# cosmodesi/desilike

Measured on AMD Instinct MI355X. Metric: log-likelihood evals/sec (full-shape P_ell, 3x40 bins), higher is better.
Workload: dtype f64; 1 GPU; BASELINE configs[1]: ShapeFit+Kaiser P_ell ell=(0,2,4) x 40 k-bins, dense window 120x1200 (n_kin=400/ell), 120x120 precision, 1024 batched param points per GPU per step; batch_per_gpu=1024, n_params=6, parallelism=walkers x1, collective=none, ranks=1

## Files before the change

### desilike_amd/csrc/dl_api.hip

```cpp
#include <hip/hip_runtime.h>
#include <chrono>
#include <thread>

#include <algorithm>
#include <cstdio>
#include <cstdlib>
#include <string>
#include <vector>

#include "../../include/desilike_amd.h"
#include "dl_host.hpp"
#include "dl_kernels.h"
#include "dl_ens_fold.h"
#include "dl_prior.h"

static thread_local std::string g_last_error;
void dl_set_last_error(const char* msg) { g_last_error = msg ? msg : ""; }

struct dl_ctx {
    int device = 0;
    int n_params = 0, n_obs = 0, n_data = 0;
    int n_white = 0;
    int N_pad = 0, K_pad = 0, K_live = 0, max_n_t = 0;
    bool any_transform = false;
// ... 389 lines not shown
        if (dl_upload(ctx, &dev, gf)) { dl_destroy(ctx); return 1; }
        ctx->gfrag_dev.push_back(dev);
    }
    ctx->obs_kernarg.resize(ctx->n_obs);
    for (int i = 0; i < ctx->n_obs; ++i) { ctx->obs[i].rebase(ctx->arena_dev); ctx->obs_kernarg[i] = ctx->obs[i].dev; }
    if (dl_upload(ctx, &ctx->obs_array_dev, ctx->obs_kernarg)) { dl_destroy(ctx); return 1; }
    {
        size_t nbytes = (16384 / 32 + 8 + 64) * sizeof(int32_t);
        if (hipMalloc((void**)&ctx->gemm_counters, nbytes) != hipSuccess || hipMemset(ctx->gemm_counters, 0, nbytes) != hipSuccess) { dl_fail(ctx, "dl_create: counter allocation failed"); dl_destroy(ctx); return 1; }
        ctx->step_ready = ctx->gemm_counters + (16384 / 32 + 8);
    }
    {
        std::vector<double> frag((size_t)ctx->N_pad * ctx->K_pad);
        const int nks = ctx->K_pad / 4;
        for (int nt = 0; nt < ctx->N_pad / 16; ++nt)
            for (int ks = 0; ks < nks; ++ks)
                for (int lane = 0; lane < 64; ++lane)
                    frag[((size_t)nt * nks + ks) * 64 + lane] = wt_white[(size_t)(16 * nt + (lane & 15)) * ctx->K_pad + 4 * ks + (lane >> 4)];
        if (dl_upload(ctx, &ctx->wt_frag_dev, frag)) { dl_destroy(ctx); return 1; }
    }
    if (dl_upload(ctx, &ctx->priors_dev, priors) || dl_upload(ctx, &ctx->wt_white_dev, wt_white) ||
        dl_upload(ctx, &ctx->bias_white_dev, bias_white) || dl_upload(ctx, &ctx->wt_full_dev, wt_full) || dl_upload(ctx, &ctx->bias_full_dev, bias_full) ||
        dl_upload(ctx, &ctx->wh_dev, wh) || dl_upload(ctx, &ctx->bias_wh_dev, bias_wh) || dl_upload(ctx, &ctx->flatdata_dev, flatdata) ||
        dl_upload(ctx, &ctx->transform_dev, transform)) {
        dl_destroy(ctx);
        return 1;
    }
    if (hipDeviceSynchronize() != hipSuccess) { dl_fail(ctx, "dl_create: hipDeviceSynchronize failed"); dl_destroy(ctx); return 1; }
    *out = ctx;
    return 0;
}

static double* dl_stk_basis_ws(dl_ctx* ctx, int i) {
    const DlObsDev& d = ctx->obs_kernarg[i];
    if (d.eng[0].type != 2 || ctx->power_ws == nullptr) return nullptr;
    const int64_t ldk = (int64_t)d.stk.n_trunks * d.eng[0].widths[d.eng[0].n_layers];
    return ldk <= (int64_t)(1 + ctx->n_var) * ctx->K_pad ? ctx->power_ws : nullptr;
}

void dl_destroy(dl_ctx* ctx) {
    if (!ctx) return;
    (void)hipSetDevice(ctx->device);
    for (double* p : {ctx->grad_wtT, ctx->grad_zero, ctx->grad_delta, ctx->grad_y, ctx->grad_phys}) if (p) (void)hipFree(p);
    for (double* p : {ctx->fa_resid, ctx->fa_jac, ctx->fa_rows}) if (p) (void)hipFree(p);
    for (double* p : {ctx->ej_basis, ctx->ej_u, ctx->ej_c, ctx->ej_dc, ctx->ej_resid, ctx->ej_rows}) if (p) (void)hipFree(p);
    for (double* p : {ctx->eg_gt, ctx->eg_u, ctx->eg_v, ctx->eg_q, ctx->eg_gb, ctx->eg_wt[0], ctx->eg_wt[1], ctx->eg_wt[2]}) if (p) (void)hipFree(p);
    if (ctx->grad_status) (void)hipFree(ctx->grad_status);
    void* ptrs[] = {ctx->arena_dev, ctx->priors_dev, ctx->wt_white_dev, ctx->wt_frag_dev, ctx->bias_white_dev, ctx->wt_full_dev, ctx->bias_full_dev, ctx->wh_dev,
                    ctx->bias_wh_dev, ctx->flatdata_dev, ctx->transform_dev, ctx->tconst_dev, ctx->power_ws, ctx->delta_ws, ctx->flat_ws, ctx->stencil_ws, ctx->theta_stage, ctx->out_stage,
                    ctx->status_stage, ctx->gemm_counters, ctx->obs_array_dev};
    for (void* p : ptrs) if (p) (void)hipFree(p);
    for (double* p : ctx->gfrag_dev) if (p) (void)hipFree(p);
    for (auto& ob : ctx->obs) if (ob.tns) { dl_tns_destroy(ob.tns); ob.tns = nullptr; }
    if (ctx->feat_ws) (void)hipFree(ctx->feat_ws);
    for (hipEvent_t e : ctx->ev) if (e) (void)hipEventDestroy(e);
    if (ctx->order_event) (void)hipEventDestroy(ctx->order_event);
    if (ctx->host_stage) (void)hipHostFree(ctx->host_stage);
    if (ctx->host_flag) (void)hipHostFree(ctx->host_flag);
    if (ctx->host_event) (void)hipEventDestroy(ctx->host_event);
    if (ctx->host_stream) (void)hipStreamDestroy(ctx->host_stream);
    delete ctx;
}

static bool dl_fisher_emu_in_scope(const dl_ctx* ctx);
static int64_t dl_fisher_emu_per_pass(const dl_ctx* ctx);

int64_t dl_info(const dl_ctx* ctx, const char* key) {
    if (!ctx || !key) return -1;
    std::string k(key);
    if (k == "fisher_analytic_pass") return dl_fisher_emu_in_scope(ctx) ? dl_fisher_emu_per_pass(ctx) : -1;
    if (k == "n_params") return ctx->n_params;
    if (k == "n_data") return ctx->n_data;
    if (k == "n_obs") return ctx->n_obs;
    if (k == "n_in_total") { int64_t t = 0; for (auto& o : ctx->obs) t += o.n_cols(); return t; }
    if (k == "K_pad") return ctx->K_pad;
    if (k == "N_pad") return ctx->N_pad;
    if (k == "n_solved") return ctx->n_solved;
    if (k == "device") return ctx->device;
    for (int i = 0; i < ctx->n_obs; ++i) {
        if (k == "n_in_obs" + std::to_string(i)) return ctx->obs[i].dev.n_in;
        if (k == "n_out_obs" + std::to_string(i)) return ctx->obs[i].n_out;
        if (k == "n_ell_obs" + std::to_string(i)) return ctx->obs[i].dev.n_ell;
        if (k == "n_kin_obs" + std::to_string(i)) return ctx->obs[i].dev.n_kin;
    }
    return -1;
}

static const int64_t DL_CHUNK = 32768;

static int dl_reserve(dl_ctx* ctx, int64_t B) {
    int64_t need = std::min<int64_t>(B, DL_CHUNK);
    if (need <= ctx->cap) return 0;
    need = std::min<int64_t>(std::max<int64_t>(need, 1024), DL_CHUNK);
    if (ctx->cap > 0) DL_HIP_CHECK(ctx, hipDeviceSynchronize());
    for (double** p : {&ctx->power_ws, &ctx->delta_ws, &ctx->flat_ws, &ctx->feat_ws, &ctx->stencil_ws}) if (*p) { (void)hipFree(*p); *p = nullptr; }
    ctx->cap = 0;
    const size_t R = 1 + ctx->n_var;
    DL_HIP_CHECK(ctx, hipMalloc((void**)&ctx->power_ws, (size_t)need * R * ctx->K_pad * sizeof(double)));
    DL_HIP_CHECK(ctx, hipMalloc((void**)&ctx->delta_ws, std::max<size_t>(2 * (size_t)need * R, (size_t)need * R + 16384 + 2048) * ctx->N_pad * sizeof(double)));
    DL_HIP_CHECK(ctx, hipMalloc((void**)&ctx->flat_ws, (size_t)need * ctx->N_pad * sizeof(double)));
    if (ctx->feat_ok) DL_HIP_CHECK(ctx, hipMalloc((void**)&ctx->feat_ws, (size_t)need * ctx->feat_ld * sizeof(double)));
    DL_HIP_CHECK(ctx, hipMalloc((void**)&ctx->stencil_ws, (size_t)need * ctx->n_params * sizeof(double)));
    DL_HIP_CHECK(ctx, hipMemset(ctx->power_ws, 0, (size_t)need * R * ctx->K_pad * sizeof(double)));
    DL_HIP_CHECK(ctx, hipMemset(ctx->delta_ws, 0, std::max<size_t>(2 * (size_t)need * R, (size_t)need * R + 16384 + 2048) * ctx->N_pad * sizeof(double)));
    DL_HIP_CHECK(ctx, hipMemset(ctx->flat_ws, 0, (size_t)need * ctx->N_pad * sizeof(double)));
    if (ctx->feat_ok) DL_HIP_CHECK(ctx, hipMemset(ctx->feat_ws, 0, (size_t)need * ctx->feat_ld * sizeof(double)));
    DL_HIP_CHECK(ctx, hipMemset(ctx->stencil_ws, 0, (size_t)need * ctx->n_params * sizeof(double)));
    DL_HIP_CHECK(ctx, hipDeviceSynchronize());
    ctx->cap = need;
    return 0;
}

static int dl_eval_impl(dl_ctx* ctx, const double* theta_dev, int64_t B, double* loglike_dev, double* logprior_dev, double* flattheory_dev, int32_t* status_dev,
                        double* solved_dev, void* hip_stream, int post_mode, double* hessian_dev = nullptr) {
    if (!ctx) { g_last_error = "dl_eval_batch: null context"; return 1; }
    if (B < 0 || (B > 0 && !theta_dev)) return dl_fail(ctx, "dl_eval_batch: invalid batch");
    if (B == 0) return 0;
    hipStream_t stream = (hipStream_t)hip_stream;
    dl_prof_events.start = dl_prof_events.stop = nullptr;
    DL_HIP_CHECK(ctx, hipSetDevice(ctx->device));
    if (dl_order_streams(ctx, stream)) return 1;
    if (dl_reserve(ctx, B)) return 1;
    const int n = ctx->n_data, P = ctx->n_params, R = 1 + ctx->n_var;
    for (int64_t b0 = 0; b0 < B; b0 += DL_CHUNK) {
        int64_t nb = std::min<int64_t>(DL_CHUNK, B - b0);
        const double* th = theta_dev + (size_t)b0 * P;
        bool prof = ctx->profile && b0 == 0 && (ctx->eval_calls % ctx->prof_every == ctx->prof_every / 2);
        hipEvent_t* ev = prof ? &ctx->ev[(size_t)(ctx->prof_calls % dl_ctx::NPOOL) * 6] : nullptr;
        const int64_t pc = ctx->prof_calls;
        const int only = !ctx->prof_rotate ? -1 : ctx->prof_only;
        if (prof) ctx->prof_phase_of[(size_t)(pc % dl_ctx::NPOOL)] = (int8_t)only;
        auto prof_phase = [&](int k) {
            const bool on = ev && k >= 0 && (only < 0 || only == k);
            dl_prof_events.start = on ? ev[2 * k] : nullptr;
            dl_prof_events.stop = on ? ev[2 * k + 1] : nullptr;
        };
        bool need_flat = ctx->any_transform || flattheory_dev != nullptr;
        const bool feat_path = ctx->feat_ok && !need_flat;
        const bool emu_fused_env = !dl_options().no_emu_fused;
        const bool emu_fused = emu_fused_env || ctx->any_stacked;
        const int64_t chi2_max_rows = dl_options().chi2_max_rows;
        const bool chi2_path = !feat_path && !ctx->any_transform && ctx->n_solved == 0 && nb <= chi2_max_rows;
        const int xcd_local = dl_options().xcd_local;
        const bool chi2_fused_env_early = dl_options().chi2_fused;
        const bool chi2_fused_early = chi2_fused_env_early && !ctx->priors_general;
        const int xcd_block = !xcd_local ? 0 : chi2_path ? (chi2_fused_early ? 32 : dl_chi2_gemm_row_tile(nb, ctx->N_pad)) : (xcd_local > 1 && !feat_path && !ctx->any_transform && ctx->n_solved == 0 && ctx->N_pad == 128) ? 64 : 0;
        const bool step_kernel_allowed = dl_options().step_kernel;
        if (step_kernel_allowed && chi2_path && !need_flat && ctx->n_obs == 1 && !ctx->priors_general && ctx->K_pad % 128 == 0 &&
            dl_step_lds_bytes(ctx->obs_kernarg[0], nb, ctx->N_pad) != 0) {
            prof_phase(0);
            dl_launch_step(ctx->obs_kernarg[0], th, P, nb, ctx->power_ws, ctx->K_pad, ctx->wt_white_dev, ctx->K_pad, ctx->bias_white_dev, ctx->delta_ws, ctx->K_pad, ctx->K_live,
                           ctx->gemm_counters, ctx->step_ready, 8, ctx->priors_dev, loglike_dev ? loglike_dev + b0 : nullptr, logprior_dev ? logprior_dev + b0 : nullptr,
                           status_dev ? status_dev + b0 : nullptr, post_mode, stream, ctx->panel_ranges.empty() ? nullptr : ctx->panel_ranges.data());
            prof_phase(-1);
            if (prof) ctx->prof_calls++;
            continue;
        }
        prof_phase(0);
        if (!(feat_path && emu_fused))
            dl_launch_fullshape(ctx->obs_kernarg.data(), ctx->n_obs, th, P, nb, ctx->power_ws, ctx->K_pad, nullptr, 0, stream, feat_path ? ctx->feat_ws : nullptr, ctx->feat_ld,
                                xcd_block, ctx->obs_array_dev);
        prof_phase(1);
        int n_slabs = 1, cps = 0;
        int64_t slab_stride = 0;
        const double* fin_bias = nullptr;
        if (need_flat) {
// ... 292 lines not shown
    if (dl_reserve(ctx, need)) return 1;
    if (need > ctx->eg_cap || !ctx->grad_status) {
        DL_HIP_CHECK(ctx, hipDeviceSynchronize());
        for (double** p : {&ctx->eg_u, &ctx->eg_v, &ctx->eg_q, &ctx->eg_gb}) if (*p) { (void)hipFree(*p); *p = nullptr; }
        if (ctx->grad_status) { (void)hipFree(ctx->grad_status); ctx->grad_status = nullptr; }
        ctx->eg_cap = 0;
        ctx->grad_cap = 0;
        const int64_t cap = std::max<int64_t>((need + 63) / 64 * 64, 256);
        DL_HIP_CHECK(ctx, hipMalloc((void**)&ctx->eg_u, (size_t)cap * K * sizeof(double)));
        DL_HIP_CHECK(ctx, hipMalloc((void**)&ctx->eg_v, (size_t)cap * K * sizeof(double)));
        DL_HIP_CHECK(ctx, hipMalloc((void**)&ctx->eg_q, (size_t)cap * (1 + ctx->n_var) * DL_N_MONO * sizeof(double)));
        DL_HIP_CHECK(ctx, hipMalloc((void**)&ctx->eg_gb, std::max<size_t>(2 * (size_t)cap, (size_t)cap + 16384 + 2048) * ctx->eg_ngt * sizeof(double)));
        DL_HIP_CHECK(ctx, hipMalloc((void**)&ctx->grad_status, (size_t)cap * sizeof(int32_t)));
        DL_HIP_CHECK(ctx, hipMemset(ctx->eg_v, 0, (size_t)cap * K * sizeof(double)));
        DL_HIP_CHECK(ctx, hipDeviceSynchronize());
        ctx->eg_cap = cap;
    }
    for (int64_t b0 = 0; b0 < B; b0 += per_pass) {
        const int64_t nb = std::min<int64_t>(per_pass, B - b0);
        const double* th = theta_dev + (size_t)b0 * P;
        int32_t* st = status_dev ? status_dev + b0 : ctx->grad_status;
        dl_launch_fullshape(ctx->obs_kernarg.data(), 1, th, P, nb, ctx->power_ws, ctx->K_pad, nullptr, 0, stream, ctx->feat_ws, ctx->feat_ld, 0, nullptr);
        dl_launch_emu_grad_u(ctx->feat_ws, ctx->feat_ld, o.feat_off, o.nb_pad, ctx->gfrag_dev[0], ctx->eg_u, Np, Np, nb, stream);
        dl_launch_emu_grad_adjoint(ctx->feat_ws, ctx->feat_ld, o.feat_off, o.nb_pad, ctx->n_var, ctx->eg_u, Np, Np, ctx->bias_white_dev, ctx->marg, th, P, ctx->priors_dev,
                                   logposterior_dev + b0, st, ctx->eg_v, ctx->eg_q, nb, stream);
        int cps = 0;
        const int n_slabs = dl_gemm_tiled_splits(nb, ctx->eg_ngt, (int)K, &cps);
        const int64_t slab_stride = nb * (int64_t)ctx->eg_ngt;
        dl_launch_window_gemm_tiled(ctx->eg_v, K, ctx->eg_gt, K, ctx->eg_gb, slab_stride, ctx->eg_ngt, nb, ctx->eg_ngt, (int)K, n_slabs, cps, stream, 0);
        dl_launch_emu_grad_backprop(o, th, P, ctx->priors_dev, ctx->eg_gb, ctx->eg_ngt, n_slabs, slab_stride, ctx->eg_q, st, ctx->eg_wt, grad_dev + (size_t)b0 * P, nb, stream);
    }
    DL_HIP_CHECK(ctx, hipGetLastError());
    return 0;
}

int dl_eval_logposterior_grad(dl_ctx* ctx, const double* theta_dev, int64_t B, double* logposterior_dev, double* grad_dev, int32_t* status_dev, void* hip_stream) {
    if (!ctx) { g_last_error = "dl_eval_logposterior_grad: null context"; return 1; }
    if (B < 0 || (B > 0 && (!theta_dev || !logposterior_dev || !grad_dev))) return dl_fail(ctx, "dl_eval_logposterior_grad: invalid argument");
    const bool emu = ctx->feat_ok && !ctx->any_transform && !ctx->priors_general && ctx->n_obs == 1 && !ctx->any_stacked &&
                     dl_emu_grad_applicable(ctx->obs_kernarg[0], ctx->N_pad, ctx->n_solved);
    if (emu) {
        if (B == 0) return 0;
        DL_HIP_CHECK(ctx, hipSetDevice(ctx->device));
        if (dl_order_streams(ctx, (hipStream_t)hip_stream)) return 1;
        return dl_eval_logposterior_grad_emu(ctx, theta_dev, B, logposterior_dev, grad_dev, status_dev, (hipStream_t)hip_stream);
    }
    if (ctx->feat_ok || ctx->any_transform || ctx->n_solved != 0 || ctx->priors_general || !dl_grad_applicable(ctx->obs_kernarg.data(), ctx->n_obs)) return 2;
    if (B == 0) return 0;
    hipStream_t stream = (hipStream_t)hip_stream;
    dl_prof_events.start = dl_prof_events.stop = nullptr;
    DL_HIP_CHECK(ctx, hipSetDevice(ctx->device));
    if (dl_order_streams(ctx, stream)) return 1;
    const int64_t per_pass = 2048;
    if (dl_reserve(ctx, std::min<int64_t>(B, per_pass))) return 1;
    const int P = ctx->n_params, Np = ctx->N_pad, Kp = ctx->K_pad;
    if (!ctx->grad_wtT) {
        std::vector<double> w((size_t)Np * Kp), wt((size_t)Kp * Np);
        DL_HIP_CHECK(ctx, hipMemcpy(w.data(), ctx->wt_white_dev, w.size() * sizeof(double), hipMemcpyDeviceToHost));
        for (int j = 0; j < Np; ++j) for (int k = 0; k < Kp; ++k) wt[(size_t)k * Np + j] = -w[(size_t)j * Kp + k];
        DL_HIP_CHECK(ctx, hipMalloc((void**)&ctx->grad_wtT, wt.size() * sizeof(double)));
        DL_HIP_CHECK(ctx, hipMemcpy(ctx->grad_wtT, wt.data(), wt.size() * sizeof(double), hipMemcpyHostToDevice));
        DL_HIP_CHECK(ctx, hipDeviceSynchronize());
    }
    const int64_t need = std::min<int64_t>(B, per_pass);
    if (need > ctx->grad_cap) {
        if (ctx->grad_cap > 0) DL_HIP_CHECK(ctx, hipDeviceSynchronize());
        for (double** p : {&ctx->grad_delta, &ctx->grad_y, &ctx->grad_phys}) if (*p) { (void)hipFree(*p); *p = nullptr; }
        if (ctx->grad_status) { (void)hipFree(ctx->grad_status); ctx->grad_status = nullptr; }
        ctx->grad_cap = 0;
        const int64_t cap = std::max<int64_t>((need + 63) / 64 * 64, 256);
        DL_HIP_CHECK(ctx, hipMalloc((void**)&ctx->grad_delta, (size_t)cap * Np * sizeof(double)));
        DL_HIP_CHECK(ctx, hipMalloc((void**)&ctx->grad_y, (size_t)cap * Kp * sizeof(double)));
        DL_HIP_CHECK(ctx, hipMalloc((void**)&ctx->grad_phys, (size_t)cap * ctx->n_obs * 8 * sizeof(double)));
        DL_HIP_CHECK(ctx, hipMalloc((void**)&ctx->grad_status, (size_t)cap * sizeof(int32_t)));
        DL_HIP_CHECK(ctx, hipMemset(ctx->grad_delta, 0, (size_t)cap * Np * sizeof(double)));
        DL_HIP_CHECK(ctx, hipDeviceSynchronize());
        ctx->grad_cap = cap;
    }
    const int xcd_local = dl_options().xcd_local;
    for (int64_t b0 = 0; b0 < B; b0 += per_pass) {
        const int64_t nb = std::min<int64_t>(per_pass, B - b0);
        const double* th = theta_dev + (size_t)b0 * P;
        int32_t* st = status_dev ? status_dev + b0 : ctx->grad_status;
        dl_launch_fullshape(ctx->obs_kernarg.data(), ctx->n_obs, th, P, nb, ctx->power_ws, ctx->K_pad, nullptr, 0, stream, nullptr, 0, xcd_local ? dl_chi2_gemm_row_tile(nb, Np) : 0, ctx->obs_array_dev);
        dl_launch_chi2_gemm(ctx->power_ws, Kp, ctx->wt_white_dev, Kp, ctx->bias_white_dev, ctx->delta_ws, nb, Np, Kp, nullptr, th, P, ctx->priors_dev, nullptr, nullptr, nullptr, 1, stream,
                            ctx->panel_ranges.empty() ? nullptr : ctx->panel_ranges.data(), ctx->K_live, ctx->grad_delta, Np, ctx->wt_frag_dev);
        dl_launch_finalize_part(ctx->delta_ws, Np / 16, th, P, ctx->priors_dev, nb, logposterior_dev + b0, nullptr, st, 1, stream);
        dl_launch_window_gemm_tiled(ctx->grad_delta, Np, ctx->grad_wtT, Np, ctx->grad_y, 0, Kp, nb, Kp, Np, 1, Np / 16, stream, 0);
        dl_launch_fullshape_grad(ctx->obs_kernarg.data(), ctx->n_obs, ctx->obs_array_dev, th, P, nb, ctx->grad_y, Kp, ctx->grad_phys, ctx->priors_dev, st, grad_dev + (size_t)b0 * P, stream);
    }
    DL_HIP_CHECK(ctx, hipGetLastError());
    return 0;
}

int dl_eval_theory(dl_ctx* ctx, const double* theta_dev, int64_t B, int32_t iobs, double* power_dev, double* tables_dev, void* hip_stream) {
    if (!ctx) { g_last_error = "dl_eval_theory: null context"; return 1; }
    if (iobs < 0 || iobs >= ctx->n_obs) return dl_fail(ctx, "dl_eval_theory: observable index out of range");
    if (B < 0 || (B > 0 && (!theta_dev || !power_dev))) return dl_fail(ctx, "dl_eval_theory: invalid argument");
    if (B == 0) return 0;
    hipStream_t stream = (hipStream_t)hip_stream;
    DL_HIP_CHECK(ctx, hipSetDevice(ctx->device));
    DlObsDev tmp = ctx->obs_kernarg[iobs];
    tmp.col_offset = 0;
    tmp.n_pass = 0;
    tmp.n_var = 0;
    for (int c = 0; c < DL_N_VPARS; ++c) tmp.vp_slot[c] = -1;
    for (int c = 0; c < DL_MAX_EFT; ++c) tmp.marg_ct_slot[c][0] = tmp.marg_ct_slot[c][1] = -1;
    if (dl_order_streams(ctx, stream)) return 1;
    dl_launch_fullshape(&tmp, 1, theta_dev, ctx->n_params, B, power_dev, tmp.n_in, tables_dev, 3 * (int64_t)tmp.n_in, stream);
    DL_HIP_CHECK(ctx, hipGetLastError());
    return 0;
}

int dl_eval_tns_tables(dl_ctx* ctx, const double* theta_dev, int64_t B, int32_t iobs, double* tables_dev, void* hip_stream) {
    if (!ctx) { g_last_error = "dl_eval_tns_tables: null context"; return 1; }
    if (iobs < 0 || iobs >= ctx->n_obs) return dl_fail(ctx, "dl_eval_tns_tables: observable index out of range");
    if (ctx->obs[iobs].dev.theory != 4) return dl_fail(ctx, "dl_eval_tns_tables: the observable's theory is not the TNS model");
    if (B < 0 || (B > 0 && (!theta_dev || !tables_dev))) return dl_fail(ctx, "dl_eval_tns_tables: invalid argument");
    if (B == 0) return 0;
    hipStream_t stream = (hipStream_t)hip_stream;
    DL_HIP_CHECK(ctx, hipSetDevice(ctx->device));
    if (dl_order_streams(ctx, stream)) return 1;
    if (dl_tns_tables(ctx->obs_kernarg[iobs], theta_dev, ctx->n_params, B, tables_dev, stream)) return dl_fail(ctx, std::string("dl_eval_tns_tables: ") + dl_last_error(nullptr));
    DL_HIP_CHECK(ctx, hipGetLastError());
    return 0;
}

static int dl_stage_reserve(dl_ctx* ctx, int64_t B) {
    if (!ctx->host_stream) DL_HIP_CHECK(ctx, hipStreamCreateWithFlags(&ctx->host_stream, hipStreamNonBlocking));
    if (B <= ctx->stage_cap) return 0;
    for (void* p : {(void*)ctx->theta_stage, (void*)ctx->out_stage}) if (p) (void)hipFree(p);
    if (ctx->host_stage) (void)hipHostFree(ctx->host_stage);
    ctx->theta_stage = ctx->out_stage = ctx->host_stage = nullptr; ctx->status_stage = nullptr; ctx->stage_cap = 0;
    int64_t cap = std::max<int64_t>(B, 64);
    DL_HIP_CHECK(ctx, hipMalloc((void**)&ctx->theta_stage, (size_t)cap * ctx->n_params * sizeof(double)));
    DL_HIP_CHECK(ctx, hipMalloc((void**)&ctx->out_stage, (size_t)cap * 3 * sizeof(double)));
    DL_HIP_CHECK(ctx, hipHostMalloc((void**)&ctx->host_stage, (size_t)cap * (ctx->n_params + 3) * sizeof(double), hipHostMallocMapped));
    DL_HIP_CHECK(ctx, hipHostGetDevicePointer((void**)&ctx->host_stage_dev, ctx->host_stage, 0));
    if (!ctx->host_flag) {
        DL_HIP_CHECK(ctx, hipHostMalloc((void**)&ctx->host_flag, 64, hipHostMallocMapped));
        DL_HIP_CHECK(ctx, hipHostGetDevicePointer((void**)&ctx->host_flag_dev, ctx->host_flag, 0));
        *ctx->host_flag = 0;
        DL_HIP_CHECK(ctx, hipEventCreateWithFlags(&ctx->host_event, hipEventDisableTiming));
    }
    ctx->stage_cap = cap;
    return 0;
}

__global__ void dl_host_flag_kernel(uint64_t* flag, uint64_t seq) {
    __threadfence_system();
    __hip_atomic_store(flag, seq, __ATOMIC_RELEASE, __HIP_MEMORY_SCOPE_SYSTEM);
}

static int dl_host_mode() { return dl_options().host_mode >= 0 ? dl_options().host_mode : 3; }

static int dl_eval_host_impl(dl_ctx* ctx, const double* theta, int64_t B, double* loglike, double* logprior, double* flattheory, int32_t* status, double* solved,
                             double* logposterior) {
    DL_HIP_CHECK(ctx, hipSetDevice(ctx->device));
    if (dl_stage_reserve(ctx, B)) return 1;
    hipStream_t stream = ctx->host_stream;
    const int P = ctx->n_params;
    int mode = dl_host_mode();
    if (mode == 3 && ctx->host_seq && (ctx->host_seq & 7) == 0) (void)hipStreamQuery(stream);
    double *flat_dev = nullptr, *solved_dev = nullptr;
    if (flattheory) DL_HIP_CHECK(ctx, hipMalloc((void**)&flat_dev, (size_t)B * ctx->n_data * sizeof(double)));
    if (solved && ctx->n_solved > 0 && hipMalloc((void**)&solved_dev, (size_t)B * ctx->n_solved * sizeof(double)) != hipSuccess) {
        if (flat_dev) (void)hipFree(flat_dev);
// ... 221 lines not shown
```

### desilike_amd/csrc/dl_fullshape.h

```cpp
#pragma once
#include <math.h>
#include <stdint.h>

#if defined(__HIPCC__)
#define DL_HD __host__ __device__ __forceinline__
#define DL_PIN4(a, b, c, d) __asm__ volatile("" : "+v"(a), "+v"(b), "+v"(c), "+v"(d) : : "memory")
#define DL_STREAM_STORE(ptr, value) __hip_atomic_store((ptr), (value), __ATOMIC_RELAXED, __HIP_MEMORY_SCOPE_AGENT)
#else
#define DL_HD inline
#define DL_PIN4(a, b, c, d)
#define DL_STREAM_STORE(ptr, value) (*(ptr) = (value))
#endif

#define DL_MAX_ELL 5
#define DL_MAX_MU 32
#define DL_MAX_EFT 8
#define DL_FS_THREADS 256
#define DL_FS_KT 192
#define DL_MAX_SEG 64
#define DL_SEG_PARTS 4
#define DL_MAX_X 16
#define DL_MAX_LAYERS 8
#define DL_MAX_WIDTH 256
#define DL_N_VPARS 11
#define DL_N_MONO 19
#define DL_STK_REC 8
#define DL_STK_MAX_GROUPS 8
#define DL_STK_MAX_MONO 5
#define DL_MAX_ML 40
#define DL_PNG_MAX_MU 48
#define DL_MAX_BAND 16
#define DL_MAX_PASS 32
#define DL_MAX_SOLVED 16
#define DL_FIR_D 28
#define DL_FIR_PAD 32
#define DL_FIR_TAPS { -0.7320508075688774, 0.4641016151377547, -0.12435565298214114, 0.033320996790809666, -0.008928334181097484, 0.002392339933580261, -0.0006410255532235571, 0.0001717622793139658, -4.602356403230609e-05, 1.2331976815258487e-05, -3.3043432287278414e-06, 8.85396099652874e-07, -2.3724116988365352e-07, 6.356857988173978e-08, -1.7033149643305495e-08, 4.564018691482174e-09, -1.2229251226231984e-09, 3.2768179901061786e-10, -8.780207341927256e-11, 2.3526494666472232e-11, -6.303905246616353e-12, 1.6891263199931699e-12, -4.5260003335632413e-13, 1.212738134321263e-13, -3.24952203721809e-14, 8.707068056597241e-15, -2.333051854208057e-15, 6.251393602349824e-16, -1.675055867318723e-16 }
#define DL_FIR_MU (-0.2679491924311228)
#define DL_FIR_LN_ABS_MU (-1.3169578969248164)
#define DL_SEG_QMAX 12

struct DlInput {
    int32_t col;
    int32_t pad;
    double value;
};

#ifdef __HIP_DEVICE_COMPILE__
DL_HD double dl_get(const DlInput& in, const double* th) { const double v = th[in.col >= 0 ? in.col : 0]; return in.col >= 0 ? v : in.value; }
#else
DL_HD double dl_get(const DlInput& in, const double* th) { return in.col >= 0 ? th[in.col] : in.value; }
#endif

struct DlObsDev {
    int32_t theory, templ, apmode, transform;
    int32_t n_ell, n_kin, n_mu, n_t;
    int32_t n_in, ell0, n_ct, n_sn;
    int32_t seg_len, seg_warm, n_seg, fixed_spline;
    int32_t uniform_knots, toeplitz;
    int64_t col_offset;
    int32_t n_var, damping_fid;
    int32_t marg_ct_slot[DL_MAX_EFT][2];
    double eta, f_fid, a, nd, x0, inv_hx;
    double end0a, end0b, end1a, end1b;
    DlInput qpar, qper, qiso, qap, df, dm, dn, sigpar, sigper, b1X, b1Y, sn0;
    DlInput to_m, to_n, qto, dpto;
    double lkto_fid, lpkto_fid;
    int32_t n_band, pad_band;
    DlInput band_in[DL_MAX_BAND];
    const double* band_tab;
    int32_t png_vel, pad_vel;
    DlInput bv, sigmau;
    double png_velfac;
    DlInput ct_in[DL_MAX_EFT][2];
    DlInput sn_in[DL_MAX_EFT];
    int32_t n_pass, bao_mode;
    const double* pass_tab;
    DlInput dbeta, sigmas;
    DlInput dres;
    double res_sig[4];
    int32_t n_ml, pad_ml;
    const double* ml_tab;
    double smoothing_radius;
    int32_t n_x, n_basis, n_mono, mono_mode;
    int32_t nb_pad, feat_pad;
    int64_t feat_off;
    DlInput x_in[DL_MAX_X];
    DlInput vp_in[DL_N_VPARS];
    int32_t vp_slot[DL_N_VPARS];
    int32_t pad2;
    double snd, fsat, sigv;
    struct Engine {
        int32_t type, n_layers, act, n_terms;
        int32_t widths[DL_MAX_LAYERS + 1];
        int32_t pad;
        double ylo, yscale, cst;
        const double *xlo, *xinv;
        const double *weights;
        const double *center, *powers, *coef;
    } eng[3];
    struct Stack {
        int32_t n_groups, n_trunks, trunk_doubles, max_k;
        int32_t frag_doubles, max_net;
        const double* wfrag;
        const double* table;
        const double* scale;
    } stk;
    const double *coef_w, *coef_n;
    const double *pknow_k;
    const double *kin, *lkin, *mu, *wmu;
    const double *x_t, *pk_fid, *sf_th, *sf_lg;
    const double *ih, *dlt;
    const double *sp_A, *sp_nC, *sp_inv;
    const double *sp_gf, *sp_gb;
    const double *coef_fixed;
    const double *ct_matrix, *sn_matrix;
    DlInput sigmav, b2, bs, b3;
    void* tns_plan;
    DlInput fnl, pX, pY, bphiX, bphiY, sigmasY;
    int32_t png_mode, pad_png;
    double png_th0, png_lg0;
    const double* png_alpha;
};

DL_HD int dl_fs_n_dd0(const DlObsDev& o) { return (o.n_var > 0 && o.n_ct > 0) ? o.n_kin : 0; }

enum {
    DL_PT_QPAR = 0, DL_PT_QPER, DL_PT_JAC, DL_PT_F, DL_PT_B1X, DL_PT_B1Y, DL_PT_SN0ND, DL_PT_DAMP,
    DL_PT_LQ = 8,
    DL_PT_FAC = DL_PT_LQ + DL_MAX_MU,
    DL_PT_SD = DL_PT_FAC + DL_MAX_MU,
    DL_PT_CT = DL_PT_SD + DL_MAX_MU,
    DL_PT_SN = DL_PT_CT + DL_MAX_EFT,
    DL_PT_OM = DL_PT_SN + DL_MAX_EFT,
    DL_PT_LQH = DL_PT_OM + 8 * DL_MAX_MU,
    DL_PT_PART = DL_PT_LQH + DL_MAX_MU,
    DL_PT_SIZE_FAST = DL_PT_PART + 2 * DL_FIR_PAD + 8,
    DL_PT_W3 = DL_PT_PART + DL_FS_THREADS,
    DL_PT_SIZE = DL_PT_W3 + 15 * DL_MAX_MU
};

struct DlFsShared {
    double* y;
    double* M;
    double* z;
    double* coef;
    double* out;
    double* pt;
};

DL_HD size_t dl_fs_work_doubles(int n_t, int n_in) { size_t w = 3 * (size_t)n_t; if (2 * (size_t)n_in > w) w = 2 * (size_t)n_in; return (w + 1) & ~(size_t)1; }
DL_HD size_t dl_fs_work_doubles(int n_t, int n_in, int n_dd0) { size_t w = 3 * (size_t)n_t; if ((size_t)n_in + n_dd0 > w) w = (size_t)n_in + n_dd0; return (w + 1) & ~(size_t)1; }
DL_HD size_t dl_fs_shared_doubles(int n_t, int n_in) { return 4 * (size_t)n_t + dl_fs_work_doubles(n_t, n_in) + DL_PT_SIZE; }
DL_HD size_t dl_fs_shared_doubles_obs(const DlObsDev& o, bool fast = false) { return 4 * (size_t)o.n_t + dl_fs_work_doubles(o.n_t, o.n_in, dl_fs_n_dd0(o)) + (fast ? DL_PT_SIZE_FAST : DL_PT_SIZE); }

DL_HD size_t dl_png_shared_doubles(int n_t, int n_in) { return dl_fs_shared_doubles(n_t, n_in) + 8 * DL_PNG_MAX_MU + 16; }

DL_HD DlFsShared dl_fs_shared_carve(double* base, int n_t, int n_in, int n_dd0 = -1, bool toep = false) {
    DlFsShared s;
    s.coef = base;
    double* work = base + 4 * (size_t)n_t;
    if (toep) { s.y = work + DL_FIR_PAD; s.M = work + (size_t)n_t + 2 * DL_FIR_PAD; s.z = s.M; }
    else { s.y = work; s.M = work + (size_t)n_t; s.z = work + 2 * (size_t)n_t; }
    s.out = work;
    s.pt = work + (n_dd0 < 0 ? dl_fs_work_doubles(n_t, n_in) : dl_fs_work_doubles(n_t, n_in, n_dd0));
    return s;
}

DL_HD void dl_ap_qparqper(const DlObsDev& o, const double* th, double& qpar, double& qper) {
    switch (o.apmode) {
        case 1: qpar = qper = dl_get(o.qiso, th); break;
        case 2: { double qap = dl_get(o.qap, th); qpar = pow(qap, 1. - o.eta); qper = pow(qap, -o.eta); break; }
        case 3: { double qiso = dl_get(o.qiso, th), qap = dl_get(o.qap, th); qpar = qiso * pow(qap, 1. - o.eta); qper = qiso * pow(qap, -o.eta); break; }
        default: qpar = dl_get(o.qpar, th); qper = dl_get(o.qper, th);
    }
}

struct DlMuCarry {
    double qpar, qper, jac, f, b1X, b1Y, sigpar, sigper;
    double mu, iq2, x;
    double fac, lq, mup2;
    double w[DL_MAX_ELL + 1];
};

DL_HD void dl_fs_mu_partA(const DlObsDev& o, const double* th, int m, DlMuCarry& c) {
    dl_ap_qparqper(o, th, c.qpar, c.qper);
    c.sigpar = dl_get(o.sigpar, th); c.sigper = dl_get(o.sigper, th);
    c.jac = 1. / (c.qpar * c.qper * c.qper);
    c.f = o.f_fid * dl_get(o.df, th);
    c.b1X = dl_get(o.b1X, th); c.b1Y = dl_get(o.b1Y, th);
    const double rq = c.qper / c.qpar;
    c.iq2 = rq * rq;
    c.mu = o.mu[m];
    for (int l = 0; l < DL_MAX_ELL; ++l) c.w[l] = o.wmu[(l < o.n_ell ? l : 0) * o.n_mu + m];
    c.w[DL_MAX_ELL] = o.wmu[(o.ell0 >= 0 ? o.ell0 : 0) * o.n_mu + m];
    c.x = 1. + c.mu * c.mu * (c.iq2 - 1.);
}

DL_HD void dl_fs_mu_partB(DlMuCarry& c) {
    c.fac = sqrt(c.x);
    c.mup2 = c.mu * c.mu * c.iq2 / c.x;
    c.lq = 0.5 * log10(c.x) - log10(c.qper);
}

DL_HD void dl_fs_mu_partC(const DlObsDev& o, const DlFsShared& s, int m, const DlMuCarry& c, bool w3 = true) {
    s.pt[DL_PT_FAC + m] = c.fac;
    s.pt[DL_PT_LQ + m] = c.lq;
    s.pt[DL_PT_LQH + m] = c.lq * o.inv_hx;
    if (o.damping_fid) {
        const double mu2 = c.mu * c.mu;
        s.pt[DL_PT_SD + m] = (c.sigpar * c.sigpar * mu2 + c.sigper * c.sigper * (1. - mu2)) * (c.qper * c.qper) / c.x;
    } else {
        s.pt[DL_PT_SD + m] = c.sigpar * c.sigpar * c.mup2 + c.sigper * c.sigper * (1. - c.mup2);
    }
    const double fm2 = c.f * c.mup2;
    const double bias = (c.b1X + fm2) * (c.b1Y + fm2);
    for (int l = 0; l < DL_MAX_ELL; ++l) {
        double w = (l < o.n_ell) ? c.jac * c.w[l] : 0.;
        s.pt[DL_PT_OM + m * 8 + l] = w * bias;
        if (w3) {
            s.pt[DL_PT_W3 + (m * 5 + l) * 3 + 0] = w;
            s.pt[DL_PT_W3 + (m * 5 + l) * 3 + 1] = w * fm2;
            s.pt[DL_PT_W3 + (m * 5 + l) * 3 + 2] = w * (fm2 * fm2);
        }
    }
    s.pt[DL_PT_OM + m * 8 + 5] = (o.ell0 >= 0) ? c.jac * c.w[DL_MAX_ELL] : 0.;
    s.pt[DL_PT_OM + m * 8 + 6] = 0.;
    s.pt[DL_PT_OM + m * 8 + 7] = 0.;
}

DL_HD void dl_fs_scalars(const DlObsDev& o, const double* th, const DlFsShared& s, const DlMuCarry& c, bool w3 = true) {
    for (int mm = o.n_mu; mm < ((o.n_mu + 3) & ~3); ++mm) {
        s.pt[DL_PT_LQ + mm] = 0.; s.pt[DL_PT_LQH + mm] = 0.; s.pt[DL_PT_FAC + mm] = 0.; s.pt[DL_PT_SD + mm] = 0.;
        for (int q = 0; q < 8; ++q) s.pt[DL_PT_OM + mm * 8 + q] = 0.;
        if (w3) for (int q = 0; q < 15; ++q) s.pt[DL_PT_W3 + mm * 15 + q] = 0.;
    }
    s.pt[DL_PT_QPAR] = c.qpar;
    s.pt[DL_PT_QPER] = c.qper;
    s.pt[DL_PT_JAC] = c.jac;
    s.pt[DL_PT_F] = c.f;
    s.pt[DL_PT_B1X] = c.b1X;
    s.pt[DL_PT_B1Y] = c.b1Y;
    s.pt[DL_PT_SN0ND] = dl_get(o.sn0, th) / o.nd;
    s.pt[DL_PT_DAMP] = (c.sigpar != 0. || c.sigper != 0.) ? 1. : 0.;
    for (int q = 0; q < o.n_ct; ++q)
        s.pt[DL_PT_CT + q] = 0.5 * (dl_get(o.ct_in[q][0], th) + dl_get(o.ct_in[q][1], th));
    for (int q = 0; q < o.n_sn; ++q)
        s.pt[DL_PT_SN + q] = dl_get(o.sn_in[q], th) / o.nd;
}

DL_HD void dl_fs_knots(int tid, int nthr, const DlObsDev& o, const double* th, const DlFsShared& s) {
    const int n_t = o.n_t;
    if (o.toeplitz && !o.fixed_spline && tid < 2 * DL_FIR_PAD) s.y[tid < DL_FIR_PAD ? tid - DL_FIR_PAD : n_t + tid - DL_FIR_PAD] = 0.;
    if (o.fixed_spline) {
        for (int j = tid; j < 4 * n_t; j += nthr) s.coef[(j & 2) * n_t + 2 * (j >> 2) + (j & 1)] = o.coef_fixed[j];
    } else if (o.templ == 1) {
        double dm_a = dl_get(o.dm, th) / o.a, dn = dl_get(o.dn, th);
        for (int j = tid; j < n_t; j += nthr) s.y[j] = o.pk_fid[j] * exp(dm_a * o.sf_th[j] + dn * o.sf_lg[j]);
    } else if (o.templ == 2) {
        const double inv_lkto = 1. / (o.lkto_fid + log10(dl_get(o.qto, th))), lp = o.lpkto_fid + log(dl_get(o.dpto, th));
        const double cm = dl_get(o.to_m, th), cn = dl_get(o.to_n, th);
        for (int j = tid; j < n_t; j += nthr) {
            const double x = o.x_t[j] * inv_lkto - 1.;
            s.y[j] = exp(lp * (1. - (x > 0. ? cm : cn) * (x * x)));
        }
    } else if (o.templ == 3) {
        const double df = dl_get(o.df, th), inv_df2 = 1. / (df * df);
        for (int j = tid; j < n_t; j += nthr) {
            double factor = 1.;
            for (int i = 0; i < o.n_band; ++i) factor += (dl_get(o.band_in[i], th) - 1.) * o.band_tab[(size_t)i * n_t + j];
            s.y[j] = o.pk_fid[j] * factor * inv_df2;
        }
    } else {
        for (int j = tid; j < n_t; j += nthr) s.y[j] = o.pk_fid[j];
    }
}

DL_HD void dl_fs_phase01(int tid, int nthr, const DlObsDev& o, const double* th, const DlFsShared& s) {
    const int mnode = nthr - 1 - tid;
    if (mnode < o.n_mu || tid == 0) {
        DlMuCarry c;
        dl_fs_mu_partA(o, th, mnode < o.n_mu ? mnode : 0, c);
        if (mnode < o.n_mu) { dl_fs_mu_partB(c); dl_fs_mu_partC(o, s, mnode, c); }
        if (tid == 0) dl_fs_scalars(o, th, s, c);
    }
    dl_fs_knots(tid, nthr, o, th, s);
}

DL_HD void dl_fs_phase2a(int tid, int nthr, const DlObsDev& o, const DlFsShared& s) {
    int m = o.n_t - 2;
    for (int i = tid; i < m; i += nthr) {
        double r = 6. * ((s.y[i + 2] - s.y[i + 1]) * o.ih[i + 1] - (s.y[i + 1] - s.y[i]) * o.ih[i]);
        s.M[i + 1] = r * o.sp_inv[i];
    }
}

DL_HD void dl_fs_phase2b_dot(int tid, int nthr, const DlObsDev& o, const DlFsShared& s) {
    const int m = o.n_t - 2;
    int seg = tid / DL_SEG_PARTS, part = tid % DL_SEG_PARTS;
    int start = seg * o.seg_len;
    double acc = 0.;
    if (start < m) {
#pragma unroll
        for (int q = 0; q < DL_SEG_QMAX; ++q) {
            int idx = start - (DL_SEG_PARTS * q + part);
            double g = o.sp_gf[q * DL_FS_THREADS + tid];
            double b = (idx >= 1) ? s.M[idx] : 0.;
            acc = fma(g, b, acc);
        }
    }
    s.pt[DL_PT_PART + tid] = acc;
}

DL_HD void dl_fs_phase2b(int tid, int nthr, const DlObsDev& o, const DlFsShared& s) {
    if (tid >= o.n_seg) return;
    const int m = o.n_t - 2;
    int start = tid * o.seg_len, end = start + o.seg_len;
    if (end > m) end = m;
    if (start >= m) return;
    const double* part = s.pt + DL_PT_PART + tid * DL_SEG_PARTS;
    double zz = (part[0] + part[1]) + (part[2] + part[3]);
#pragma unroll 8
    for (int i = start; i < end; ++i) {
        zz = fma(o.sp_A[i], zz, s.M[i + 1]);
        s.z[i] = zz;
    }
}

DL_HD void dl_fs_phase2c_dot(int tid, int nthr, const DlObsDev& o, const DlFsShared& s) {
    const int m = o.n_t - 2;
    int seg = tid / DL_SEG_PARTS, part = tid % DL_SEG_PARTS;
    int start = seg * o.seg_len, end = start + o.seg_len;
    if (end > m) end = m;
    double acc = 0.;
    if (start < m) {
#pragma unroll
        for (int q = 0; q < DL_SEG_QMAX; ++q) {
            int idx = end + DL_SEG_PARTS * q + part;
            double g = o.sp_gb[q * DL_FS_THREADS + tid];
            double zv = (idx < m) ? s.z[idx] : 0.;
            acc = fma(g, zv, acc);
        }
    }
    s.pt[DL_PT_PART + tid] = acc;
}

DL_HD void dl_fs_phase2c(int tid, int nthr, const DlObsDev& o, const DlFsShared& s) {
    if (tid >= o.n_seg) return;
    const int m = o.n_t - 2;
    int start = tid * o.seg_len, end = start + o.seg_len;
    if (end > m) end = m;
    if (start >= m) return;
    const double* part = s.pt + DL_PT_PART + tid * DL_SEG_PARTS;
    double uu = (part[0] + part[1]) + (part[2] + part[3]);
#pragma unroll 8
    for (int i = end - 1; i >= start; --i) {
        uu = fma(o.sp_nC[i], uu, s.z[i]);
        s.M[i + 1] = uu;
    }
}

DL_HD void dl_fs_phase2d(int tid, int nthr, const DlObsDev& o, const DlFsShared& s) {
    const int n = o.n_t;
    const double hx = 1. / o.inv_hx;
    for (int j = tid; j < n - 1; j += nthr) {
        double Ml = (j == 0) ? (o.end0a * s.M[1] + o.end0b * s.M[2]) : s.M[j];
        double Mr = (j == n - 2) ? (o.end1a * s.M[n - 2] + o.end1b * s.M[n - 3]) : s.M[j + 1];
        double ihj = o.ih[j];
        double h = o.x_t[j + 1] - o.x_t[j];
        double yl = s.y[j], yr = s.y[j + 1];
        double c0 = yl;
        double c1 = (yr - yl) * ihj - h * (2. * Ml + Mr) * (1. / 6.);
        double c2 = 0.5 * Ml;
        double c3 = (Mr - Ml) * ihj * (1. / 6.);
        double d0, d1, d2, d3;
        if (o.uniform_knots) {
            double dl = -o.dlt[j];
            d0 = c0 + dl * (c1 + dl * (c2 + dl * c3));
            d1 = hx * (c1 + dl * (2. * c2 + 3. * dl * c3));
            d2 = hx * hx * (c2 + 3. * dl * c3);
            d3 = hx * hx * hx * c3;
        } else {
            d0 = c0; d1 = c1 * h; d2 = c2 * h * h; d3 = c3 * h * h * h;
        }
        s.coef[2 * j + 0] = d0; s.coef[2 * j + 1] = d1; s.coef[2 * n + 2 * j + 0] = d2; s.coef[2 * n + 2 * j + 1] = d3;
    }
}

DL_HD void dl_fs_phase2_fir(int tid, int nthr, const DlObsDev& o, const DlFsShared& s) {
    const double T[DL_FIR_D + 1] = DL_FIR_TAPS;
    const int n = o.n_t;
    const double scale = 6. * o.inv_hx * o.inv_hx;
    for (int j0 = 4 * tid; j0 < n; j0 += 4 * nthr) {
        double acc[4] = {0., 0., 0., 0.};
        const double* yp = s.y + j0 - DL_FIR_D;
        double cur[4], nxt[4];
#pragma unroll
        for (int c = 0; c < 4; ++c) cur[c] = yp[c];
#pragma unroll
        for (int gq = 0; gq < (2 * DL_FIR_D + 4) / 4; ++gq) {
            if (gq + 1 < (2 * DL_FIR_D + 4) / 4) {
#pragma unroll
                for (int c = 0; c < 4; ++c) nxt[c] = yp[4 * (gq + 1) + c];
            }
#pragma unroll
            for (int c = 0; c < 4; ++c) {
                const int p = 4 * gq + c;
#pragma unroll
                for (int q = 0; q < 4; ++q) {
                    const int e = p - DL_FIR_D - q;
                    if (e >= -DL_FIR_D && e <= DL_FIR_D) acc[q] = fma(T[e < 0 ? -e : e], cur[c], acc[q]);
                }
            }
            DL_PIN4(acc[0], acc[1], acc[2], acc[3]);
#pragma unroll
            for (int c = 0; c < 4; ++c) cur[c] = nxt[c];
        }
#pragma unroll
        for (int q = 0; q < 4; ++q)
            if (j0 + q < n) s.M[j0 + q] = acc[q] * scale;
    }
    for (int k = tid - (nthr - 2 * DL_FIR_PAD - 1); k >= 0 && k <= 2 * DL_FIR_PAD; k += nthr) {
        double v = exp((double)k * DL_FIR_LN_ABS_MU);
        s.pt[DL_PT_PART + k] = (k & 1) ? -v : v;
    }
}

DL_HD double dl_fir_mu_pow(const DlFsShared& s, int k) {
    return (k <= 2 * DL_FIR_PAD) ? s.pt[DL_PT_PART + k] : 0.;
}

#define DL_TOEP_PREF 3
DL_HD void dl_fs_phase2d_toep(int tid, int nthr, const DlObsDev& o, const DlFsShared& s, const double* dlt_pref) {
    const int n = o.n_t;
    const double hx = 1. / o.inv_hx, ihx = o.inv_hx;
    const double sc6 = o.inv_hx * o.inv_hx;
    const double a = sc6 * ((s.y[0] - s.y[1]) - (s.y[1] - s.y[2])) - s.M[1];
    const double b = sc6 * ((s.y[n - 3] - s.y[n - 2]) - (s.y[n - 2] - s.y[n - 1])) - s.M[n - 2];
    int it = 0;
    for (int j = tid; j < n - 1; j += nthr, ++it) {
        auto moment = [&](int i) { return s.M[i] + a * dl_fir_mu_pow(s, i - 1) + b * dl_fir_mu_pow(s, n - 2 - i); };
        double Ml, Mr;
        if (j == 0) { double m1 = moment(1), m2 = moment(2); Ml = o.end0a * m1 + o.end0b * m2; Mr = m1; }
        else if (j == n - 2) { double m1 = moment(n - 2), m2 = moment(n - 3); Ml = m1; Mr = o.end1a * m1 + o.end1b * m2; }
        else { Ml = moment(j); Mr = moment(j + 1); }
        const double yl = s.y[j], yr = s.y[j + 1];
        const double c0 = yl;
        const double c1 = (yr - yl) * ihx - hx * (2. * Ml + Mr) * (1. / 6.);
        const double c2 = 0.5 * Ml;
        const double c3 = (Mr - Ml) * ihx * (1. / 6.);
        const double dl = -(it < DL_TOEP_PREF ? dlt_pref[it] : o.dlt[j]);
        s.coef[2 * j + 0] = c0 + dl * (c1 + dl * (c2 + dl * c3));
        s.coef[2 * j + 1] = hx * (c1 + dl * (2. * c2 + 3. * dl * c3));
        s.coef[2 * n + 2 * j + 0] = hx * hx * (c2 + 3. * dl * c3);
        s.coef[2 * n + 2 * j + 1] = hx * hx * hx * c3;
    }
}

template <bool UNIF>
DL_HD void dl_spline_locate(const DlObsDev& o, double x, int& j, double& u) {
    const int n = o.n_t;
    if (UNIF || o.uniform_knots) {
        double t = (x - o.x0) * o.inv_hx;
        double tc = t > 0. ? t : 0.;
        j = (int)tc;
        if (j > n - 2) j = n - 2;
        u = t - (double)j;
    } else {
        int lo = 0, hi = n - 1;
        while (hi - lo > 1) {
            int mid = (lo + hi) >> 1;
            if (x >= o.x_t[mid]) lo = mid; else hi = mid;
        }
        j = lo;
        u = (x - o.x_t[j]) * o.ih[j];
    }
}

template <bool UNIF>
DL_HD double dl_spline_eval(const DlObsDev& o, const DlFsShared& s, double x) {
    int j;
    double u;
    dl_spline_locate<UNIF>(o, x, j, u);
    const double* c = s.coef + 2 * j;
    const double* d = c + 2 * o.n_t;
    return fma(fma(fma(d[1], u, d[0]), u, c[1]), u, c[0]);
}

DL_HD double dl_spline_eval_t(const DlObsDev& o, const DlFsShared& s, double t) {
    int j = (int)t;
#if defined(__HIP_DEVICE_COMPILE__)
    __asm__("v_med3_i32 %0, %1, 0, %2" : "=v"(j) : "v"(j), "s"(o.n_t - 2));
#else
    j = j < 0 ? 0 : j;
    if (j > o.n_t - 2) j = o.n_t - 2;
#endif
    const double u = t - (double)j;
    const double* c = s.coef + 2 * j;
    const double* d = c + 2 * o.n_t;
    return fma(fma(fma(d[1], u, d[0]), u, c[1]), u, c[0]);
}

#define DL_P3_PREF 2
template <bool FAST, int NL, bool EFT>
DL_HD void dl_fs_phase3(int tid, int nthr, const DlObsDev& o, const DlFsShared& s, double* tables_row, const double* lk_pref = nullptr) {
    const double qper = s.pt[DL_PT_QPER], sn0nd = s.pt[DL_PT_SN0ND];
    const double b1X = s.pt[DL_PT_B1X], b1Y = s.pt[DL_PT_B1Y];
    const bool damp = s.pt[DL_PT_DAMP] != 0.;
    const bool need_dd0 = EFT && o.n_ct > 0;
    const bool TABLES = !FAST && tables_row != nullptr;
    const int n_ell = o.n_ell, n_kin = o.n_kin;
    const int n_mu4 = (o.n_mu + 3) & ~3;
    int it = 0;
    for (int i = tid; i < n_kin; i += nthr, ++it) {
        const double lk = (lk_pref != nullptr && it < DL_P3_PREF) ? lk_pref[it] : o.lkin[i];
        const double kq = damp ? o.kin[i] / qper : 0.;
        double p[NL];
        double dd[FAST ? 1 : NL], dt[FAST ? 1 : NL], tt[FAST ? 1 : NL];
        double dd0 = 0.;
#pragma unroll
        for (int l = 0; l < NL; ++l) p[l] = 0.;
#pragma unroll
        for (int l = 0; l < (FAST ? 1 : NL); ++l) dd[l] = dt[l] = tt[l] = 0.;
        for (int m0 = 0; m0 < n_mu4; m0 += 4) {
            double T[4];
#pragma unroll
            for (int q = 0; q < 4; ++q) T[q] = dl_spline_eval<FAST>(o, s, lk + s.pt[DL_PT_LQ + m0 + q]);
            if (damp) {
#pragma unroll
                for (int q = 0; q < 4; ++q) {
                    double kap = kq * s.pt[DL_PT_FAC + m0 + q];
                    T[q] *= exp(-(kap * kap * s.pt[DL_PT_SD + m0 + q]) / 2.);
                }
            }
            if (FAST || !TABLES) {
#pragma unroll
                for (int q = 0; q < 4; ++q) {
                    const double* om = s.pt + DL_PT_OM + (m0 + q) * 8;
#pragma unroll
                    for (int l = 0; l < NL; ++l) p[l] = fma(om[l], T[q], p[l]);
                    if (need_dd0) dd0 = fma(om[5], T[q], dd0);
                }
            } else {
#pragma unroll
                for (int q = 0; q < 4; ++q) {
                    const double* w3 = s.pt + DL_PT_W3 + (m0 + q) * 15;
#pragma unroll
                    for (int l = 0; l < (FAST ? 1 : NL); ++l) {
                        dd[l] = fma(w3[3 * l + 0], T[q], dd[l]);
                        dt[l] = fma(w3[3 * l + 1], T[q], dt[l]);
                        tt[l] = fma(w3[3 * l + 2], T[q], tt[l]);
                    }
                }
            }
        }
        if (!FAST && TABLES) {
#pragma unroll
            for (int l = 0; l < (FAST ? 1 : NL); ++l) {
                if (l < n_ell) {
                    p[l] = b1X * b1Y * dd[l] + (b1X + b1Y) * dt[l] + tt[l];
                    if (l == o.ell0) dd0 = dd[l];
                    tables_row[(size_t)(0 * n_ell + l) * n_kin + i] = dd[l];
                    tables_row[(size_t)(1 * n_ell + l) * n_kin + i] = dt[l];
                    tables_row[(size_t)(2 * n_ell + l) * n_kin + i] = tt[l];
                }
            }
        }
#pragma unroll
        for (int l = 0; l < NL; ++l) {
            if (l < n_ell) {
                double pl = p[l] + (l == o.ell0 ? sn0nd : 0.);
                if (EFT && o.n_ct > 0) {
                    double acc = 0.;
                    for (int c = 0; c < o.n_ct; ++c) acc += o.ct_matrix[((size_t)l * n_kin + i) * o.n_ct + c] * s.pt[DL_PT_CT + c];
                    pl += acc * dd0;
                }
                if (EFT && o.n_sn > 0) {
                    double acc = 0.;
                    for (int c = 0; c < o.n_sn; ++c) acc += o.sn_matrix[((size_t)l * n_kin + i) * o.n_sn + c] * s.pt[DL_PT_SN + c];
                    pl += acc;
                }
                s.out[(size_t)l * n_kin + i] = pl;
            }
        }
        if (EFT && o.n_var > 0) s.out[o.n_in + i] = dd0;
    }
}

template <int NL, bool EFT>
DL_HD void dl_fs_phase3_pair(int tid, int nthr, const DlObsDev& o, const DlFsShared& s, const double* lk_pref = nullptr) {
    const double qper = s.pt[DL_PT_QPER], sn0nd = s.pt[DL_PT_SN0ND];
    const bool damp = s.pt[DL_PT_DAMP] != 0.;
    const bool need_dd0 = EFT && o.n_ct > 0;
    const int n_ell = o.n_ell, n_kin = o.n_kin;
    const int n_mu4 = (o.n_mu + 3) & ~3;
    auto finish = [&](int i, const double* p, double dd0) {
#pragma unroll
        for (int l = 0; l < NL; ++l) {
            if (l < n_ell) {
                double pl = p[l] + (l == o.ell0 ? sn0nd : 0.);
                if (EFT && o.n_ct > 0) {
                    double acc = 0.;
                    for (int c = 0; c < o.n_ct; ++c) acc += o.ct_matrix[((size_t)l * n_kin + i) * o.n_ct + c] * s.pt[DL_PT_CT + c];
                    pl += acc * dd0;
                }
                if (EFT && o.n_sn > 0) {
                    double acc = 0.;
                    for (int c = 0; c < o.n_sn; ++c) acc += o.sn_matrix[((size_t)l * n_kin + i) * o.n_sn + c] * s.pt[DL_PT_SN + c];
                    pl += acc;
                }
                s.out[(size_t)l * n_kin + i] = pl;
            }
        }
        if (EFT && o.n_var > 0) s.out[o.n_in + i] = dd0;
    };
    int it = 0;
    for (int i = tid; i < n_kin; i += 2 * nthr, it += 2) {
        const int i2 = i + nthr;
        const bool two = i2 < n_kin;
        const double lkA = (((lk_pref != nullptr && it < DL_P3_PREF) ? lk_pref[it] : o.lkin[i]) - o.x0) * o.inv_hx;
        const double lkB = !two ? lkA : (((lk_pref != nullptr && it + 1 < DL_P3_PREF) ? lk_pref[it + 1] : o.lkin[i2]) - o.x0) * o.inv_hx;
        const double kqA = damp ? o.kin[i] / qper : 0.;
        const double kqB = (damp && two) ? o.kin[i2] / qper : 0.;
        double pA[NL], pB[NL];
        double dd0A = 0., dd0B = 0.;
#pragma unroll
        for (int l = 0; l < NL; ++l) pA[l] = pB[l] = 0.;
        for (int m0 = 0; m0 < n_mu4; m0 += 4) {
            double lq[4], TA[4], TB[4];
#pragma unroll
            for (int q = 0; q < 4; ++q) lq[q] = s.pt[DL_PT_LQH + m0 + q];
#pragma unroll
            for (int q = 0; q < 4; ++q) TA[q] = dl_spline_eval_t(o, s, lkA + lq[q]);
            if (two) {
#pragma unroll
                for (int q = 0; q < 4; ++q) TB[q] = dl_spline_eval_t(o, s, lkB + lq[q]);
            } else {
#pragma unroll
                for (int q = 0; q < 4; ++q) TB[q] = 0.;
            }
            if (damp) {
#pragma unroll
                for (int q = 0; q < 4; ++q) {
                    const double fac = s.pt[DL_PT_FAC + m0 + q], sd = s.pt[DL_PT_SD + m0 + q];
                    double kap = kqA * fac;
                    TA[q] *= exp(-(kap * kap * sd) / 2.);
                    if (two) { kap = kqB * fac; TB[q] *= exp(-(kap * kap * sd) / 2.); }
                }
            }
#pragma unroll
            for (int q = 0; q < 4; ++q) {
                const double* om = s.pt + DL_PT_OM + (m0 + q) * 8;
#pragma unroll
                for (int l = 0; l < NL; ++l) {
                    const double w = om[l];
                    pA[l] = fma(w, TA[q], pA[l]);
                    pB[l] = fma(w, TB[q], pB[l]);
                }
                if (need_dd0) { const double w = om[5]; dd0A = fma(w, TA[q], dd0A); dd0B = fma(w, TB[q], dd0B); }
            }
        }
        finish(i, pA, dd0A);
        if (two) finish(i2, pB, dd0B);
    }
}

DL_HD void dl_fs_phase4(int tid, int nthr, const DlObsDev& o, const DlFsShared& s, const double* th, double* power_row, int64_t ld) {
    for (int idx = tid; idx < o.n_in; idx += nthr) DL_STREAM_STORE(&power_row[idx], s.out[idx]);
    for (int c = tid; c < o.n_pass; c += nthr) { const int col = (int)o.pass_tab[2 * c]; power_row[o.n_in + c] = col >= 0 ? th[col] : o.pass_tab[2 * c + 1]; }
    if (o.n_var > 0 && o.n_ct > 0) {
        for (int c = 0; c < o.n_ct; ++c) {
            for (int t = 0; t < 2; ++t) {
                int slot = o.marg_ct_slot[c][t];
                if (slot < 0) continue;
                if (t == 1 && o.marg_ct_slot[c][0] == slot) continue;
                double wgt = (o.marg_ct_slot[c][0] == o.marg_ct_slot[c][1]) ? 1. : 0.5;
                double* drow = power_row + (size_t)(1 + slot) * ld;
                for (int idx = tid; idx < o.n_in; idx += nthr) {
                    int i = idx % o.n_kin;
                    drow[idx] = wgt * o.ct_matrix[(size_t)idx * o.n_ct + c] * s.out[o.n_in + i];
                }
            }
        }
    }
}

DL_HD void dl_png_setup(int tid, int nthr, const DlObsDev& o, const double* th, double* murec, double* sc) {
    if (tid == nthr - 1) {
        double qpar, qper;
        dl_ap_qparqper(o, th, qpar, qper);
        const double b1X = dl_get(o.b1X, th), b1Y = dl_get(o.b1Y, th), fnl = dl_get(o.fnl, th);
        sc[0] = qper; sc[1] = 1. / (qpar * qper * qper); sc[2] = o.f_fid * dl_get(o.df, th); sc[3] = b1X; sc[4] = b1Y;
        sc[5] = o.png_mode == 0 ? dl_get(o.bphiX, th) * fnl : 2. * 1.686 * (b1X - dl_get(o.pX, th)) * fnl;
        sc[6] = o.png_mode == 0 ? dl_get(o.bphiY, th) * fnl : 2. * 1.686 * (b1Y - dl_get(o.pY, th)) * fnl;
        const double sX = dl_get(o.sigmas, th), sY = dl_get(o.sigmasY, th);
        sc[7] = 0.5 * sX * sX; sc[8] = 0.5 * sY * sY; sc[9] = dl_get(o.sn0, th) / o.nd;
        sc[10] = dl_get(o.bv, th) * sc[2] * o.png_velfac; sc[11] = dl_get(o.sigmau, th);
    }
    if (tid >= nthr - 1 - o.n_mu && tid < nthr - 1) {
        const int m = nthr - 2 - tid;
        double qpar, qper;
        dl_ap_qparqper(o, th, qpar, qper);
        const double mu = o.mu[m], rq = qper / qpar;
        const double x = 1. + mu * mu * (rq * rq - 1.);
        murec[8 * m] = 0.5 * log10(x) - log10(qper);
        murec[8 * m + 1] = sqrt(x);
        murec[8 * m + 2] = mu * mu * rq * rq / x;
        murec[8 * m + 3] = o.n_ell > 4 ? o.wmu[4 * o.n_mu + m] : 0.;
        for (int l = 0; l < 4; ++l) murec[8 * m + 4 + l] = l < o.n_ell ? o.wmu[l * o.n_mu + m] : 0.;
    }
}

DL_HD void dl_png_knots(int tid, int nthr, const DlObsDev& o, const double* th, const DlFsShared& s, bool alpha) {
    const int n_t = o.n_t;
    const double dm_a = dl_get(o.dm, th) / o.a, dn = dl_get(o.dn, th);
    if (o.toeplitz && tid < 2 * DL_FIR_PAD) s.y[tid < DL_FIR_PAD ? tid - DL_FIR_PAD : n_t + tid - DL_FIR_PAD] = 0.;
    const double norm = (alpha && o.templ == 1) ? exp(dm_a * o.png_th0 + dn * o.png_lg0) : 1.;
    for (int j = tid; j < n_t; j += nthr) {
        const double fac = o.templ == 1 ? exp(dm_a * o.sf_th[j] + dn * o.sf_lg[j]) : 1.;
// ... 572 lines not shown
```

### desilike_amd/csrc/dl_host.hpp

```cpp
#pragma once
#include <algorithm>
#include <cmath>
#include <cstdlib>
#include <cstdint>
#include <cstring>
#include <map>
#include <string>
#include <vector>

#include "dl_fullshape.h"
#include "dl_tns.h"

struct dl_config {
    std::map<std::string, std::vector<double>> f64;
    std::map<std::string, std::vector<int32_t>> i32;

    bool has_f64(const std::string& k) const { return f64.count(k) > 0; }
    bool has_i32(const std::string& k) const { return i32.count(k) > 0; }
    const std::vector<double>& F(const std::string& k) const {
        static const std::vector<double> empty;
        auto it = f64.find(k);
        return it == f64.end() ? empty : it->second;
    }
    const std::vector<int32_t>& I(const std::string& k) const {
        static const std::vector<int32_t> empty;
        auto it = i32.find(k);
        return it == i32.end() ? empty : it->second;
    }
    double f(const std::string& k, double def) const { auto& v = F(k); return v.empty() ? def : v[0]; }
    int32_t i(const std::string& k, int32_t def) const { auto& v = I(k); return v.empty() ? def : v[0]; }
};

struct DlArena {
    std::vector<double> data;
    size_t push(const double* src, size_t n) {
        size_t off = data.size();
        data.insert(data.end(), src, src + n);
        if (data.size() % 2) data.push_back(0.);
        return off;
    }
    size_t push(const std::vector<double>& v) { return push(v.data(), v.size()); }
};

struct DlTnsPlan;
struct DlObsHost {
    DlObsDev dev;
    DlTnsPlan* tns = nullptr;
    std::vector<double> tns_k11, tns_mu, tns_wmu, tns_kt;
    int tns_fog = 0;
    int n_out = 0;
    int marg_sn0 = -1;
    int marg_sn[DL_MAX_EFT];
    int marg_ct[DL_MAX_EFT][2];
    std::vector<double> weff;
    std::vector<double> bias;
    std::vector<double> flatdata;
    size_t off_kin, off_lkin, off_mu, off_wmu, off_xt, off_pk, off_th, off_lg, off_ih, off_dlt, off_A, off_nC, off_inv, off_gf, off_gb, off_coef, off_ct, off_sn;
    size_t off_cw, off_cn, off_pknowk, off_ml, off_pass, off_png = 0, off_band = 0;
    size_t off_eng[3][6];
    size_t off_stk[3] = {0, 0, 0};
    int marg_vp[DL_N_VPARS];
    int marg_pass[DL_MAX_PASS];
    int n_cols() const { return dev.n_in + dev.n_pass; }

    void rebase(const double* base) {
        dev.kin = base + off_kin; dev.lkin = base + off_lkin; dev.mu = base + off_mu; dev.wmu = base + off_wmu;
        dev.x_t = base + off_xt; dev.pk_fid = base + off_pk; dev.sf_th = base + off_th; dev.sf_lg = base + off_lg;
        dev.ih = base + off_ih; dev.dlt = base + off_dlt; dev.sp_A = base + off_A; dev.sp_nC = base + off_nC; dev.sp_inv = base + off_inv;
        dev.sp_gf = base + off_gf; dev.sp_gb = base + off_gb; dev.coef_fixed = base + off_coef;
        dev.ct_matrix = base + off_ct; dev.sn_matrix = base + off_sn;
        dev.coef_w = base + off_cw; dev.coef_n = base + off_cn; dev.pknow_k = base + off_pknowk; dev.ml_tab = base + off_ml; dev.pass_tab = base + off_pass; dev.png_alpha = base + off_png; dev.band_tab = base + off_band;
        for (int e = 0; e < 3; ++e) {
            dev.eng[e].xlo = base + off_eng[e][0]; dev.eng[e].xinv = base + off_eng[e][1]; dev.eng[e].weights = base + off_eng[e][2];
            dev.eng[e].center = base + off_eng[e][3]; dev.eng[e].powers = base + off_eng[e][4]; dev.eng[e].coef = base + off_eng[e][5];
        }
        dev.stk.table = base + off_stk[0]; dev.stk.scale = base + off_stk[1]; dev.stk.wfrag = base + off_stk[2];
    }
};

struct DlSplineSetup {
    std::vector<double> ih, A, nC, inv;
    double end0a, end0b, end1a, end1b;
    int warm;
};

inline bool dl_spline_setup(const std::vector<double>& x, DlSplineSetup& s, std::string& err) {
    int n = (int)x.size();
    if (n < 5) { err = "spline needs at least 5 knots"; return false; }
    std::vector<double> h(n - 1);
    s.ih.resize(n - 1);
    for (int j = 0; j < n - 1; ++j) {
        h[j] = x[j + 1] - x[j];
        if (!(h[j] > 0.)) { err = "template knots must be strictly increasing"; return false; }
        s.ih[j] = 1. / h[j];
    }
    int m = n - 2;
    std::vector<double> lo(m), di(m), up(m);
    for (int i = 0; i < m; ++i) {
        lo[i] = h[i];
        di[i] = 2. * (h[i] + h[i + 1]);
        up[i] = h[i + 1];
    }
    s.end0a = 1. + h[0] / h[1];
    s.end0b = -h[0] / h[1];
    di[0] += h[0] * s.end0a;
    up[0] += h[0] * s.end0b;
    lo[0] = 0.;
    s.end1a = 1. + h[n - 2] / h[n - 3];
    s.end1b = -h[n - 2] / h[n - 3];
    di[m - 1] += h[n - 2] * s.end1a;
    lo[m - 1] += h[n - 2] * s.end1b;
    up[m - 1] = 0.;
    s.A.resize(m); s.nC.resize(m); s.inv.resize(m);
    double cprev = 0.;
    double amax = 0.;
    for (int i = 0; i < m; ++i) {
        double den = di[i] - lo[i] * cprev;
        if (!(std::fabs(den) > 0.)) { err = "singular spline system"; return false; }
        s.inv[i] = 1. / den;
        s.A[i] = -lo[i] * s.inv[i];
        cprev = up[i] * s.inv[i];
        s.nC[i] = -cprev;
        amax = std::fmax(amax, std::fmax(std::fabs(s.A[i]), std::fabs(cprev)));
    }
    if (amax < 0.9 && amax > 0.) s.warm = (int)std::ceil(std::log(1e-19) / std::log(amax)) + 1;
    else s.warm = m;
    if (s.warm > m) s.warm = m;
    return true;
}

inline void dl_spline_moments_serial(const std::vector<double>& y, const DlSplineSetup& s, std::vector<double>& M) {
    int n = (int)y.size(), m = n - 2;
    std::vector<double> z(m);
    M.assign(n, 0.);
    double zz = 0.;
    for (int i = 0; i < m; ++i) {
        double r = 6. * ((y[i + 2] - y[i + 1]) * s.ih[i + 1] - (y[i + 1] - y[i]) * s.ih[i]);
        zz = std::fma(s.A[i], zz, r * s.inv[i]);
        z[i] = zz;
    }
    double uu = 0.;
    for (int i = m - 1; i >= 0; --i) {
        uu = std::fma(s.nC[i], uu, z[i]);
        M[i + 1] = uu;
    }
    M[0] = s.end0a * M[1] + s.end0b * M[2];
    M[n - 1] = s.end1a * M[n - 2] + s.end1b * M[n - 3];
}

inline DlInput dl_input_from(const dl_config& cfg, const std::string& key, double def) {
    DlInput in;
    in.col = -1; in.pad = 0; in.value = def;
// ... 241 lines not shown
    const auto& pk = cfg.F(p + "pk_dd_fid");
    d.n_ell = (int)ells.size(); d.n_kin = (int)kin.size(); d.n_mu = (int)mu.size(); d.n_t = (int)k_t.size();
    d.n_in = d.n_ell * d.n_kin;
    if (d.n_ell < 1 || d.n_ell > DL_MAX_ELL) { err = p + "ells_in: between 1 and 5 multipoles supported"; return false; }
    if (d.n_mu < 1 || d.n_mu > (d.theory == 5 ? DL_PNG_MAX_MU : DL_MAX_MU)) { err = p + "mu: between 1 and 32 nodes supported (48 by the PNG theory)"; return false; }
    if (d.n_kin < 1) { err = p + "kin missing"; return false; }
    if ((int)wmu.size() != d.n_ell * d.n_mu) { err = p + "wmu_ell must have n_ell * n_mu entries"; return false; }
    if ((int)pk.size() != d.n_t) { err = p + "pk_dd_fid and k_t sizes differ"; return false; }
    d.ell0 = -1;
    for (int l = 0; l < d.n_ell; ++l) if (ells[l] == 0) d.ell0 = l;
    d.eta = cfg.f(p + "eta", 1. / 3.);
    d.f_fid = cfg.f(p + "f_fid", 1.);
    d.a = cfg.f(p + "a", 0.6);
    double kp = cfg.f(p + "kp", 0.03);
    d.nd = cfg.f(p + "nd", 1e-4);
    struct { const char* name; DlInput* in; double def; } inputs[] = {
        {"qpar", &d.qpar, 1.}, {"qper", &d.qper, 1.}, {"qiso", &d.qiso, 1.}, {"qap", &d.qap, 1.}, {"df", &d.df, 1.}, {"dm", &d.dm, 0.}, {"dn", &d.dn, 0.},
        {"sigmapar", &d.sigpar, 0.}, {"sigmaper", &d.sigper, 0.}, {"b1X", &d.b1X, 1.}, {"b1Y", &d.b1Y, 1.}, {"sn0", &d.sn0, 0.},
        {"dbeta", &d.dbeta, 1.}, {"sigmas", &d.sigmas, 0.}, {"dres", &d.dres, 1.},
        {"sigmav", &d.sigmav, 0.}, {"b2", &d.b2, 0.}, {"bs", &d.bs, 0.}, {"b3", &d.b3, 0.},
        {"bv", &d.bv, 1.}, {"sigmau", &d.sigmau, 0.},
        {"m", &d.to_m, 0.6}, {"n", &d.to_n, 0.9}, {"qto", &d.qto, 1.}, {"dpto", &d.dpto, 1.},
        {"fnl_loc", &d.fnl, 0.}, {"pX", &d.pX, 1.}, {"pY", &d.pY, 1.}, {"bphiX", &d.bphiX, 1.}, {"bphiY", &d.bphiY, 1.}, {"sigmasY", &d.sigmasY, 0.}};
    for (auto& it : inputs) {
        *it.in = dl_input_from(cfg, p + "in." + it.name, it.def);
        if (it.in->col >= n_params) { err = p + "in." + it.name + ": theta column out of range"; return false; }
    }
    std::vector<double> pass_tab;
    {
        const auto& pin = cfg.F(p + "in.pass");
        d.n_pass = (int)(pin.size() / 2);
        if (d.n_pass > DL_MAX_PASS) { err = p + "at most 32 pass-through (broadband) parameters supported"; return false; }
        const auto& mpass = cfg.I(p + "marg.pass");
        for (int c = 0; c < DL_MAX_PASS; ++c) oh.marg_pass[c] = (c < (int)mpass.size()) ? mpass[c] : -1;
        pass_tab.assign(std::max<size_t>(pin.size(), 2), 0.);
        for (int c = 0; c < d.n_pass; ++c) {
            pass_tab[2 * c] = (double)std::lround(pin[2 * c]); pass_tab[2 * c + 1] = pin[2 * c + 1];
            if ((int)pass_tab[2 * c] >= n_params) { err = p + "in.pass: theta column out of range"; return false; }
        }
        d.bao_mode = cfg.i(p + "bao_mode", 0);
        d.smoothing_radius = cfg.f(p + "smoothing_radius", 15.);
        const auto& res = cfg.F(p + "resummed");
        for (int q = 0; q < 4; ++q) d.res_sig[q] = q < (int)res.size() ? res[q] : 0.;
    }
    if (d.templ == 2) {
        const double kto = cfg.f(p + "kto_fid", 0.), pkto = cfg.f(p + "pkto_fid", 0.);
        if (!(kto > 0.) || !(pkto > 0.)) { err = p + "turn-over template: kto_fid and pkto_fid must be positive"; return false; }
        if (d.theory != 0 && d.theory != 1) { err = p + "turn-over template: Kaiser / EFT-like Kaiser / Simple theories only"; return false; }
        d.lkto_fid = std::log10(kto); d.lpkto_fid = std::log(pkto);
    } else if (d.templ == 3) {
        const auto& bin = cfg.F(p + "in.band");
        const auto& btab = cfg.F(p + "band_templates");
        d.n_band = (int)(bin.size() / 2);
        if (d.n_band < 1 || d.n_band > DL_MAX_BAND) { err = p + "band template: 1 .. 16 bands (in.band)"; return false; }
        if ((int)btab.size() != d.n_band * d.n_t) { err = p + "band template: band_templates must be [n_band, n_t]"; return false; }
        if (d.theory != 0 && d.theory != 1) { err = p + "band template: Kaiser / EFT-like Kaiser / Simple theories only"; return false; }
        for (int i = 0; i < d.n_band; ++i) {
            d.band_in[i].col = (int)std::lround(bin[2 * i]); d.band_in[i].value = bin[2 * i + 1];
            if (d.band_in[i].col >= n_params) { err = p + "in.band: theta column out of range"; return false; }
        }
    } else if (d.templ < 0 || d.templ > 3) { err = p + "unknown template kind"; return false; }
    std::vector<double> x_t(d.n_t), sf_th(d.n_t), sf_lg(d.n_t), lkin(d.n_kin);
    for (int j = 0; j < d.n_t; ++j) {
        x_t[j] = std::log10(k_t[j]);
        sf_lg[j] = std::log(k_t[j] / kp);
        sf_th[j] = std::tanh(d.a * std::log(k_t[j] / kp));
    }
    for (int i = 0; i < d.n_kin; ++i) lkin[i] = std::log10(kin[i]);
    DlSplineSetup sp;
    if (!dl_spline_setup(x_t, sp, err)) { err = p + err; return false; }
    d.end0a = sp.end0a; d.end0b = sp.end0b; d.end1a = sp.end1a; d.end1b = sp.end1b;
    d.x0 = x_t[0];
    d.inv_hx = (d.n_t - 1) / (x_t[d.n_t - 1] - x_t[0]);
    d.fixed_spline = (d.templ == 0) && d.theory != 5;
    std::vector<double> dlt(d.n_t);
    d.uniform_knots = 1;
    for (int j = 0; j < d.n_t; ++j) {
        dlt[j] = x_t[j] - (d.x0 + j / d.inv_hx);
        if (std::fabs(dlt[j] * d.inv_hx) > 1e-6) d.uniform_knots = 0;
    }
    d.toeplitz = (d.uniform_knots && d.n_t >= 4 * DL_FIR_PAD && !getenv("DL_NO_TOEPLITZ")) ? 1 : 0;
    for (int j = 0; j + 1 < d.n_t && d.toeplitz; ++j)
        if (std::fabs((x_t[j + 1] - x_t[j]) * d.inv_hx - 1.) > 1e-11) d.toeplitz = 0;
    int m = d.n_t - 2;
    d.seg_warm = sp.warm;
    d.n_seg = DL_MAX_SEG;
    d.seg_len = (m + d.n_seg - 1) / d.n_seg;
    if (d.seg_warm > DL_SEG_PARTS * DL_SEG_QMAX) { err = p + "template knots too irregular for the segmented spline solve (sweep multipliers decay too slowly)"; return false; }
    std::vector<double> gf((size_t)DL_SEG_QMAX * DL_FS_THREADS, 0.), gb((size_t)DL_SEG_QMAX * DL_FS_THREADS, 0.);
    auto slot = [](int dd, int sgm) { return (size_t)(dd / DL_SEG_PARTS) * DL_FS_THREADS + (size_t)sgm * DL_SEG_PARTS + (dd % DL_SEG_PARTS); };
    for (int sgm = 0; sgm < d.n_seg; ++sgm) {
        int start = sgm * d.seg_len, end = std::min(start + d.seg_len, m);
        if (start >= m) continue;
        double g = 1.;
        for (int dd = 0; dd < d.seg_warm && start - 1 - dd >= 0; ++dd) {
            gf[slot(dd, sgm)] = g;
            g *= sp.A[start - 1 - dd];
        }
        g = 1.;
        for (int dd = 0; dd < d.seg_warm && end + dd < m; ++dd) {
            gb[slot(dd, sgm)] = g;
            g *= sp.nC[end + dd];
        }
    }
    std::vector<double> Mfix, coef((size_t)4 * d.n_t, 0.);
    dl_spline_moments_serial(pk, sp, Mfix);
    {
        std::vector<double> lds(dl_fs_shared_doubles(d.n_t, d.n_in), 0.);
        DlFsShared sh = dl_fs_shared_carve(lds.data(), d.n_t, d.n_in);
        for (int j = 0; j < d.n_t; ++j) { sh.y[j] = pk[j]; sh.M[j] = Mfix[j]; }
        DlObsDev tmp = d;
        tmp.ih = sp.ih.data(); tmp.x_t = x_t.data(); tmp.dlt = dlt.data();
        dl_fs_phase2d(0, 1, tmp, sh);
        for (int j = 0; j < d.n_t; ++j)
            for (int q = 0; q < 4; ++q) coef[(size_t)4 * j + q] = sh.coef[(size_t)(q >> 1) * 2 * d.n_t + 2 * j + (q & 1)];
    }
    std::vector<double> coef_w(4, 0.), coef_n(4, 0.), pknow_k(2, 0.);
    if (d.theory == 2) {
        const auto& pknow = cfg.F(p + "pknow_dd_fid");
        if ((int)pknow.size() != d.n_t) { err = p + "pknow_dd_fid (no-wiggle table) is required by the BAO model"; return false; }
        auto interval_polynomials = [&](const std::vector<double>& y, std::vector<double>& out) {
            std::vector<double> Mv;
            dl_spline_moments_serial(y, sp, Mv);
            std::vector<double> lds(dl_fs_shared_doubles(d.n_t, d.n_in), 0.);
            DlFsShared sh = dl_fs_shared_carve(lds.data(), d.n_t, d.n_in);
            for (int j = 0; j < d.n_t; ++j) { sh.y[j] = y[j]; sh.M[j] = Mv[j]; }
            DlObsDev tmp = d;
            tmp.ih = sp.ih.data(); tmp.x_t = x_t.data(); tmp.dlt = dlt.data();
            dl_fs_phase2d(0, 1, tmp, sh);
            out.assign((size_t)4 * d.n_t, 0.);
            for (int j = 0; j < d.n_t; ++j)
                for (int q = 0; q < 4; ++q) out[(size_t)4 * j + q] = sh.coef[(size_t)(q >> 1) * 2 * d.n_t + 2 * j + (q & 1)];
        };
        std::vector<double> wig(d.n_t);
        for (int j = 0; j < d.n_t; ++j) wig[j] = pk[j] - pknow[j];
        interval_polynomials(wig, coef_w);
        interval_polynomials(pknow, coef_n);
        pknow_k.assign(d.n_kin, 0.);
        DlObsDev tmp = d;
        tmp.ih = sp.ih.data(); tmp.x_t = x_t.data();
        for (int i = 0; i < d.n_kin; ++i) {
            int j; double u;
            dl_spline_locate<false>(tmp, lkin[i], j, u);
            const double* c = &coef_n[(size_t)4 * j];
            pknow_k[i] = std::fma(std::fma(std::fma(c[3], u, c[2]), u, c[1]), u, c[0]);
        }
    }
    const bool flexible = d.theory == 2 && cfg.has_f64(p + "ml_matrix");
    std::vector<double> ml_tab;
    if (flexible) {
        const auto& mlin = cfg.F(p + "in.ml");
        const auto& mlell = cfg.I(p + "ml_ell");
        d.n_ml = (int)mlell.size();
        if (d.n_ml > DL_MAX_ML) { err = p + "at most 40 multiplicative wiggle terms supported"; return false; }
        if ((int)mlin.size() != 2 * d.n_ml || (int)cfg.F(p + "ml_matrix").size() != d.n_ml * d.n_kin || (int)cfg.F(p + "legendre").size() != d.n_ell * d.n_mu) {
            err = p + "ml_matrix / ml_ell / in.ml / legendre sizes do not match"; return false;
        }
        for (int q = 0; q < d.n_ml; ++q) {
            const int col = (int)std::lround(mlin[2 * q]);
            if (col >= n_params || mlell[q] < 0 || mlell[q] >= d.n_ell) { err = p + "in.ml / ml_ell out of range"; return false; }
            ml_tab.push_back((double)col); ml_tab.push_back(mlin[2 * q + 1]); ml_tab.push_back((double)mlell[q]);
        }
    }
    const auto& ctm = flexible ? cfg.F(p + "ml_matrix") : cfg.F(p + "ct_matrix");
    const auto& snm = flexible ? cfg.F(p + "legendre") : cfg.F(p + "sn_matrix");
    d.n_ct = (flexible || ctm.empty()) ? 0 : (int)(ctm.size() / d.n_in);
    d.n_sn = (flexible || snm.empty()) ? 0 : (int)(snm.size() / d.n_in);
    if (d.n_ct > DL_MAX_EFT || d.n_sn > DL_MAX_EFT) { err = p + "at most 8 counter / stochastic terms supported"; return false; }
    if (d.n_ct > 0 && d.ell0 < 0) { err = p + "counter terms need the monopole in ells_in (full_shape.py:633)"; return false; }
    const auto& ctin = cfg.F(p + "in.ct");
    const auto& snin = cfg.F(p + "in.sn");
    if ((int)ctin.size() != d.n_ct * 4 || (int)snin.size() != d.n_sn * 2) { err = p + "in.ct / in.sn sizes do not match the matrices"; return false; }
    for (int c = 0; c < d.n_ct; ++c)
        for (int t = 0; t < 2; ++t) {
            d.ct_in[c][t].col = (int32_t)std::lround(ctin[(c * 2 + t) * 2]);
            d.ct_in[c][t].value = ctin[(c * 2 + t) * 2 + 1];
            if (d.ct_in[c][t].col >= n_params) { err = p + "in.ct: theta column out of range"; return false; }
        }
    for (int c = 0; c < d.n_sn; ++c) {
        d.sn_in[c].col = (int32_t)std::lround(snin[c * 2]);
        d.sn_in[c].value = snin[c * 2 + 1];
        if (d.sn_in[c].col >= n_params) { err = p + "in.sn: theta column out of range"; return false; }
    }
    {
        const auto& msn0 = cfg.I(p + "marg.sn0");
        const auto& msn = cfg.I(p + "marg.sn");
        const auto& mct = cfg.I(p + "marg.ct");
        oh.marg_sn0 = msn0.empty() ? -1 : msn0[0];
        for (int c = 0; c < DL_MAX_EFT; ++c) {
            oh.marg_sn[c] = (c < (int)msn.size()) ? msn[c] : -1;
            for (int t = 0; t < 2; ++t) { oh.marg_ct[c][t] = (2 * c + t < (int)mct.size()) ? mct[2 * c + t] : -1; d.marg_ct_slot[c][t] = -1; }
        }
        d.n_var = 0;
    }
    oh.off_kin = arena.push(kin); oh.off_lkin = arena.push(lkin); oh.off_mu = arena.push(mu); oh.off_wmu = arena.push(wmu);
    oh.off_xt = arena.push(x_t); oh.off_pk = arena.push(pk); oh.off_th = arena.push(sf_th); oh.off_lg = arena.push(sf_lg);
    oh.off_ih = arena.push(sp.ih); oh.off_dlt = arena.push(dlt); oh.off_A = arena.push(sp.A); oh.off_nC = arena.push(sp.nC); oh.off_inv = arena.push(sp.inv);
    oh.off_gf = arena.push(gf); oh.off_gb = arena.push(gb); oh.off_coef = arena.push(coef);
    oh.off_ct = arena.push(ctm); oh.off_sn = arena.push(snm);
    oh.off_cw = arena.push(coef_w); oh.off_cn = arena.push(coef_n); oh.off_pknowk = arena.push(pknow_k);
    std::vector<double> png_alpha(2, 0.);
    if (d.theory == 5) {
        const auto& al = cfg.F(p + "png_alpha");
        if ((int)al.size() != d.n_t) { err = p + "png_alpha (alpha at the template knots) is required by the PNG theory"; return false; }
        if (d.n_ct > 0 || d.n_sn > 0 || d.n_pass > 0) { err = p + "counter / stochastic / pass-through terms are not part of the PNG theory"; return false; }
        png_alpha = al;
        d.png_mode = cfg.i(p + "png_mode", 1);
        d.png_vel = cfg.i(p + "png_velocity", 0);
        d.png_velfac = cfg.f(p + "png_velfac", 100.);
        const auto& nk = cfg.F(p + "png_knorm");
        if (!nk.empty()) { d.png_lg0 = std::log(nk[0] / kp); d.png_th0 = std::tanh(d.a * d.png_lg0); }
    }
    if (ml_tab.empty()) ml_tab.assign(3, 0.);
    oh.off_ml = arena.push(ml_tab);
    oh.off_pass = arena.push(pass_tab);
    oh.off_png = arena.push(png_alpha);
    {
        std::vector<double> band_tab = d.templ == 3 ? cfg.F(p + "band_templates") : std::vector<double>(2, 0.);
        oh.off_band = arena.push(band_tab);
    }

    for (int c = 0; c < DL_N_VPARS; ++c) { oh.marg_vp[c] = -1; d.vp_slot[c] = -1; }
    for (int e = 0; e < 3; ++e) { d.eng[e].type = -1; for (int q = 0; q < 6; ++q) oh.off_eng[e][q] = oh.off_kin; }
    if (d.theory == 4) {
        const auto& k11 = cfg.F(p + "tns_k11");
        const auto& tmu = cfg.F(p + "tns_mu");
        const auto& twmu = cfg.F(p + "tns_wmu");
        if (k11.empty() || tmu.empty() || tmu.size() != twmu.size()) { err = p + "tns_k11 / tns_mu / tns_wmu are required by the TNS theory"; return false; }
        if (d.n_pass != 0) { err = p + "pass-through columns are not supported by the TNS theory"; return false; }
        if (dl_tns_assemble_doubles((int)k11.size(), d.n_in, d.n_kin, 1) * sizeof(double) > 156 * 1024) { err = p + "TNS table grid too large for the LDS of the assembly kernel (about 550 table wavenumbers)"; return false; }
        oh.tns_k11 = k11; oh.tns_mu = tmu; oh.tns_wmu = twmu; oh.tns_kt = k_t; oh.tns_fog = cfg.i(p + "tns_fog", 0);
#ifdef __HIPCC__
        const char* terr = nullptr;
        oh.tns = dl_tns_create(k11.data(), (int)k11.size(), k_t.data(), d.n_t, tmu.data(), twmu.data(), (int)tmu.size(), oh.tns_fog, &terr);
        if (!oh.tns) { err = p + (terr ? terr : "tns: plan creation failed"); return false; }
        d.tns_plan = oh.tns;
#else
        d.tns_plan = &oh;
#endif
    }
    return dl_build_window(cfg, p, oh, err);
}
```

### desilike_amd/csrc/dl_kernels.h

```cpp
#pragma once
#include <hip/hip_runtime.h>
#include <hip/hip_ext.h>
#include <stdint.h>

#include "dl_fullshape.h"

struct DlProfEvents { hipEvent_t start = nullptr, stop = nullptr; };
extern thread_local DlProfEvents dl_prof_events;
#define DL_LAUNCH(kernel, grid, block, shm, stream, ...)                                                                                       \
    do {                                                                                                                                       \
        if (dl_prof_events.start) hipExtLaunchKernelGGL(kernel, grid, block, shm, stream, dl_prof_events.start, dl_prof_events.stop, 0, __VA_ARGS__); \
        else hipLaunchKernelGGL(kernel, grid, block, shm, stream, __VA_ARGS__);                                                                \
    } while (0)

struct DlOptions {
    bool no_merged_theory, no_emu_batch, no_fused_solve, no_gram_plain, no_scaled_row0, ef_no_early_theta, fm_no_lane_solve;
    bool chi2_bfrag;
    bool no_stk_split;
    int stk_overlap;
    bool ens_global, ens_force_comm, ens_no_defer, ens_no_fold, ens_stamps, ens_fold_stamps;
    bool no_emu_fused, no_gram_epilogue, step_kernel, chi2_fused, no_chi2_big;
    int xcd_local;
    long long chi2_max_rows;
    int cg_mt;
    int host_mode;
};
const DlOptions& dl_options();

#define DL_ST_OK 0
#define DL_ST_OUT_OF_PRIOR 1
#define DL_ST_NONFINITE 2
#define DL_ST_NAN_INPUT 3

void dl_launch_fullshape(const DlObsDev* obs_host, int n_obs, const double* theta, int n_params, int64_t B, double* power, int64_t ld_power, double* tables,
                         int64_t ld_tables, hipStream_t stream, double* feat = nullptr, int64_t feat_ld = 0, int xcd_block = 0,
                         const DlObsDev* obs_dev = nullptr);
void dl_launch_window_gemm(const double* A, int64_t lda, const double* Wt, int64_t ldw, const double* bias, double* C, int64_t ldc, int64_t M, int N_valid, int N_pad,
                           int K_pad, int bias_period, hipStream_t stream);

#define DL_MARG_NJ 8
struct DlMargDev {
    int32_t n_s, n_marg;
    int32_t is_marg[DL_MAX_SOLVED];
    int32_t var_slot[DL_MAX_SOLVED];
    double x0[DL_MAX_SOLVED], loc[DL_MAX_SOLVED], prec[DL_MAX_SOLVED];
    const double* tconst;
};
void dl_launch_finalize_marg(const double* dtilde, int64_t ld, int n, int rows_per_point, int n_slabs, int64_t slab_stride, const double* bias, const DlMargDev& mg,
                             const double* theta, int n_params, const double* priors, int64_t B, double* loglike, double* logprior, int32_t* status, double* solved,
                             double* hessian , int post_mode, hipStream_t stream, bool xcd_tile16 = false,
                             const double* gram = nullptr);
void dl_launch_transform(double* flat, int64_t ld, const double* data, const int32_t* transform, int n, int64_t B, hipStream_t stream);
int dl_gemm_tiled_splits(int64_t M, int N_pad, int K_pad, int* chunks_per_split);
void dl_launch_window_gemm_tiled(const double* A, int64_t lda, const double* Wt, int64_t ldw, double* slabs, int64_t slab_stride, int64_t ldc, int64_t M, int N_pad, int K_pad,
                                 int n_splits, int chunks_per_split, hipStream_t stream, int n_live = 0);
void dl_launch_finalize(const double* dtilde, int64_t ld, int n, int n_slabs, int64_t slab_stride, const double* bias, const double* theta, int n_params,
                        const double* priors, int64_t B, double* loglike, double* logprior, int32_t* status, int post_mode, hipStream_t stream);
int dl_chi2_gemm_row_tile(int64_t M, int N_pad);
void dl_launch_chi2_gemm(const double* A, int64_t lda, const double* Wt, int64_t ldw, const double* bias, double* part, int64_t M, int N_pad, int K_pad, int32_t* counters,
                         const double* theta, int n_params, const double* priors, double* loglike, double* logprior, int32_t* status, int post_mode, hipStream_t stream,
                         const uint8_t* panel_ranges = nullptr, int k_live = 0, double* resid = nullptr, int64_t ldr = 0, const double* wfrag = nullptr);
void dl_launch_finalize_part(const double* part, int n_tiles, const double* theta, int n_params, const double* priors, int64_t B, double* loglike, double* logprior,
                             int32_t* status, int post_mode, hipStream_t stream);
#ifndef DL_FG_NM
#define DL_FG_NM 19
#define DL_FG_MONO_LD 20
#endif
void dl_launch_feature_gemm(const double* feat, int64_t feat_ld, int64_t feat_off, int nb_pad, int R, const double* gfrag, double* out, int64_t ldo, int N_pad, int64_t B,
                            int accumulate, hipStream_t stream);
int dl_gemm_dma_chi2_parts(int N_pad);
void dl_launch_window_gemm_dma_chi2(const double* A, int64_t lda, const double* Wt, int64_t ldw, const double* bias, double* part, int64_t M, int N_pad, int K_pad, hipStream_t stream, int n_live = 0);
void dl_launch_emulated_feature(const DlObsDev& obs, const double* theta, int n_params, int64_t B, const double* gfrag, double* out, int64_t ldo, int N_pad, int accumulate,
                                hipStream_t stream);
size_t dl_step_lds_bytes(const DlObsDev& obs, int64_t B, int N_pad);
void dl_launch_step(const DlObsDev& obs, const double* theta, int n_params, int64_t B, double* power, int64_t ld_power, const double* Wt, int64_t ldw, const double* bias,
                    double* part, int K_pad, int k_live, int32_t* counters, int32_t* ready, int32_t target, const double* priors, double* loglike, double* logprior, int32_t* status,
                    int post_mode, hipStream_t stream, const uint8_t* panel_ranges);
bool dl_emulated_stacked_ok(const DlObsDev& obs);
struct DlGramFinalize;
void dl_launch_emulated_stacked(const DlObsDev& obs, const double* theta, int n_params, int64_t B, const double* gfrag, double* out, int64_t ldo, int N_pad, int accumulate,
                                int steps_per_block, hipStream_t stream, DlGramFinalize* fin = nullptr, const double* bias = nullptr, const DlMargDev* mg = nullptr, int n_valid = 0,
                                double* basis_ws = nullptr, bool chains_done = false);
bool dl_launch_stk_chains(const DlObsDev& obs, const double* theta, int n_params, int64_t B, double* basis_ws, hipStream_t stream);
struct DlGramFinalize {
    const double* priors;
    double *loglike, *logprior;
    int32_t* status;
    double *solved, *hessian;
    int post_mode;
    bool done;
};
bool dl_launch_emulated_feature_gram(const DlObsDev& obs, const double* theta, int n_params, int64_t B, const double* gfrag, const double* bias, const DlMargDev& mg, int n_valid,
                                     double* gram, hipStream_t stream, DlGramFinalize* fin = nullptr);
void dl_launch_fisher_stencil(const double* centers, const double* steps, int P, int64_t B, double* theta, hipStream_t stream);
int dl_fisher_waves(int n, int P, size_t* shm_bytes, int* chunk);
void dl_launch_fisher(const double* rows, int64_t ld, int n, int n_slabs, int64_t slab_stride, const double* bias, const double* steps, int P, int64_t B, double* hessian,
                      double* gradient, double* offset, hipStream_t stream);
struct dl_ctx;
int dl_internal_eval_partials(dl_ctx* ctx, const double* theta_dev, int64_t B, const double** part, int* n_tiles, const double** priors, hipStream_t stream);
struct DlEnsFold;
int dl_internal_fold_info(dl_ctx* ctx, int64_t B, int* n_tiles, const double** priors);
int dl_internal_eval_fold(dl_ctx* ctx, const DlEnsFold& fold, int64_t B, double* part_out, hipStream_t stream);
bool dl_launch_fullshape_ens(const DlObsDev* obs_host, int n_obs, const DlObsDev* obs_dev, const DlEnsFold& f, int64_t B, double* power, int64_t ld_power, int xcd_block, hipStream_t stream);
bool dl_grad_applicable(const DlObsDev* obs_host, int n_obs);
void dl_launch_fullshape_grad(const DlObsDev* obs_host, int n_obs, const DlObsDev* obs_dev, const double* theta, int n_params, int64_t B, const double* Y, int64_t ldy, double* gphys,
                              const double* priors, const int32_t* status, double* grad, hipStream_t stream);
void dl_launch_fullshape_jac(const DlObsDev* obs_host, int n_obs, const DlObsDev* obs_dev, const double* theta, int n_params, int64_t B, int k_live, int k_pad, double* jac, int64_t ldj,
                             hipStream_t stream);
void dl_launch_fisher_rows(const double* resid, int64_t ldr, const double* drows, int64_t ld, int n, int n_slabs, int64_t slab_stride, int P, int64_t B, double* hessian,
                           double* gradient, double* offset, hipStream_t stream);
bool dl_emu_grad_applicable(const DlObsDev& obs, int N_pad, int n_solved);
void dl_launch_emu_grad_u(const double* feat, int64_t feat_ld, int64_t feat_off, int nb_pad, const double* gfrag, double* U, int64_t ldu, int N_pad, int64_t B, hipStream_t stream);
void dl_launch_emu_grad_adjoint(const double* feat, int64_t feat_ld, int64_t feat_off, int nb_pad, int n_var, const double* U, int64_t ldu, int N_pad, const double* bias,
                                const DlMargDev& mg, const double* theta, int n_params, const double* priors, double* logpost, int32_t* status, double* V, double* Q,
                                int64_t B, hipStream_t stream);
void dl_launch_emu_grad_backprop(const DlObsDev& obs, const double* theta, int n_params, const double* priors, const double* gb, int64_t ldg, int n_slabs, int64_t slab_stride,
                                 const double* Q, const int32_t* status, const double* const* wT , double* grad, int64_t B,
                                 hipStream_t stream);
bool dl_emu_jac_applicable(const DlObsDev& obs, int N_pad, int n_params);
// ... 6 lines not shown
```

### desilike_amd/csrc/dl_kernels.hip

```cpp
#include <hip/hip_runtime.h>

#include <algorithm>
#include <cstdio>
#include <cstdlib>
#include <cstring>
#include <vector>

#include "dl_fullshape.h"
#include <mutex>
#include "dl_kernels.h"
#include "dl_tns.h"
#include "dl_emu_batch.h"
#include "dl_emu_stacked.h"
#include "dl_emu_stacked_ov.h"
#include "dl_emu_stacked_split.h"
#include "dl_finalize_part.h"
#include "dl_marg_solve.h"
#include "dl_scalar_prefetch.h"
#include "dl_ens_fold.h"
#include "dl_fullshape_grad.h"
#include "dl_fullshape_jac.h"

thread_local DlProfEvents dl_prof_events;

__device__ __forceinline__ void dl_obs_prefetch(const void* p) {
    if (__builtin_amdgcn_readfirstlane(threadIdx.x) >= 64) return;
    dl_scalar_prefetch<0, (offsetof(DlObsDev, ct_in) + 63) / 64 * 64, offsetof(DlObsDev, coef_w) / 64 * 64, (sizeof(DlObsDev) + 63) / 64 * 64>(p);
}

static DlOptions g_options;
static std::once_flag g_options_once;
static void dl_options_read() {
    auto on = [](const char* name) { return std::getenv(name) != nullptr; };
    DlOptions& o = g_options;
    o.no_merged_theory = on("DL_NO_MERGED_THEORY"); o.no_emu_batch = on("DL_NO_EMU_BATCH"); o.no_fused_solve = on("DL_NO_FUSED_SOLVE"); o.no_gram_plain = on("DL_NO_GRAM_PLAIN");
    o.no_scaled_row0 = on("DL_NO_SCALED_ROW0"); o.ef_no_early_theta = on("DL_EF_NO_EARLY_THETA"); o.fm_no_lane_solve = on("DL_FM_NO_LANE_SOLVE");
    o.no_stk_split = on("DL_NO_STK_SPLIT");
    o.stk_overlap = std::getenv("DL_STK_OVERLAP") ? atoi(std::getenv("DL_STK_OVERLAP")) : 0;
    o.ens_global = on("DL_ENS_GLOBAL"); o.ens_force_comm = on("DL_ENS_FORCE_COMM"); o.ens_no_defer = on("DL_ENS_NO_DEFER"); o.ens_no_fold = on("DL_ENS_NO_FOLD");
    o.ens_stamps = on("DL_ENS_STAMPS"); o.ens_fold_stamps = on("DL_ENS_FOLD_STAMPS");
    o.cg_mt = std::getenv("DL_CG_MT") ? atoi(std::getenv("DL_CG_MT")) : 0;
    o.host_mode = std::getenv("DL_HOST_MODE") ? atoi(std::getenv("DL_HOST_MODE")) : -1;
    auto flag = [](const char* name) { const char* v = std::getenv(name); return v != nullptr && atoi(v) != 0; };
    o.no_emu_fused = on("DL_NO_EMU_FUSED"); o.no_gram_epilogue = on("DL_NO_GRAM_EPILOGUE"); o.no_chi2_big = on("DL_NO_CHI2_BIG");
    o.step_kernel = flag("DL_STEP_KERNEL"); o.chi2_fused = flag("DL_CHI2_FUSED"); o.chi2_bfrag = flag("DL_CHI2_BFRAG");
    o.xcd_local = std::getenv("DL_XCD_LOCAL") ? atoi(std::getenv("DL_XCD_LOCAL")) : 1;
    o.chi2_max_rows = std::getenv("DL_CHI2_GEMM_MAX") ? atoll(std::getenv("DL_CHI2_GEMM_MAX")) : 2048;
}
const DlOptions& dl_options() {
    std::call_once(g_options_once, dl_options_read);
    return g_options;
}
extern "C" void dl_options_refresh(void) { (void)dl_options(); dl_options_read(); }

__device__ __forceinline__ int dl_fs_point_of_wg(int wg, int xblk) { return xblk ? xblk * ((wg & 7) + 8 * ((wg >> 3) / xblk)) + ((wg >> 3) % xblk) : wg; }

template <bool FAST, int NL, bool EFT, bool DENSE, bool TH_ROW = false, bool SUB = false, int NT = DL_FS_THREADS>
__device__ __forceinline__ void dl_fullshape_body(const DlObsDev& o, const double* __restrict__ theta, int n_params, double* __restrict__ power,
                                                  int64_t ld_power, double* __restrict__ tables, int64_t ld_tables, int stop_after, unsigned long long* __restrict__ stamps,
                                                  const double* th_row = nullptr,
                                                  double* lds_sub = nullptr, int tid_sub = 0, int b_sub = 0) {
    extern __shared__ __attribute__((aligned(16))) double lds_wg[];
    double* lds = SUB ? lds_sub : lds_wg;
    const int xblk = SUB ? 0 : (stop_after >> 8) & 0xff;
    stop_after = (SUB || xblk) ? 0 : stop_after;
    const int b = SUB ? b_sub : dl_fs_point_of_wg(blockIdx.x, xblk);
#define DL_STAMP(slot) if (stamps != nullptr && threadIdx.x == 0) stamps[(size_t)blockIdx.x * 8 + (slot)] = __builtin_amdgcn_s_memtime();
    DL_STAMP(0)
    if (stamps != nullptr && threadIdx.x == 0) stamps[(size_t)blockIdx.x * 8 + 6] = __builtin_amdgcn_s_memrealtime();
    const bool toep = !o.fixed_spline && (FAST || o.toeplitz);
    const DlFsShared s = dl_fs_shared_carve(lds, o.n_t, o.n_in, dl_fs_n_dd0(o), toep);
    const double* th = TH_ROW ? th_row : theta + (size_t)b * n_params;
    const int tid = SUB ? tid_sub : (int)threadIdx.x, nthr = NT;
    if (stop_after == -1) return;
    double lk_pref[DL_P3_PREF];
#pragma unroll
    for (int it = 0; it < DL_P3_PREF; ++it) lk_pref[it] = (tid + it * nthr < o.n_kin) ? o.lkin[tid + it * nthr] : 0.;
    if (FAST) {
        constexpr int KT = NT - 64;
        const bool mu_wave = tid >= KT;
        const int m = tid - KT;
        const bool mu_lane = mu_wave && m < o.n_mu, scalar_lane = (tid == nthr - 1);
        DlMuCarry c;
        double dlt_pref[DL_TOEP_PREF];
#pragma unroll
        for (int it = 0; it < DL_TOEP_PREF; ++it) dlt_pref[it] = (toep && !mu_wave && tid + it * KT < o.n_t - 1) ? o.dlt[tid + it * KT] : 0.;
        if (mu_wave) dl_fs_mu_partA(o, th, mu_lane ? m : 0, c);
        else dl_fs_knots(tid, KT, o, th, s);
        if (o.fixed_spline && mu_wave) {
            dl_fs_mu_partB(c);
            if (mu_lane) dl_fs_mu_partC(o, s, m, c, false);
            if (scalar_lane) dl_fs_scalars(o, th, s, c, false);
        }
        __syncthreads();
        DL_STAMP(1)
        if (stop_after == 1) return;
        if (toep) {
            if (mu_wave) dl_fs_mu_partB(c);
            else dl_fs_phase2_fir(tid, KT, o, s);
            __syncthreads();
            DL_STAMP(2)
            if (stop_after == 2) return;
            if (mu_wave) {
                if (mu_lane) dl_fs_mu_partC(o, s, m, c, false);
                if (scalar_lane) dl_fs_scalars(o, th, s, c, false);
            } else dl_fs_phase2d_toep(tid, KT, o, s, dlt_pref);
            __syncthreads();
            DL_STAMP(3)
            if (stop_after == 5) return;
        }
    } else {
        dl_fs_phase01(tid, nthr, o, th, s);
        __syncthreads();
        if (stop_after == 1) return;
        if (toep) {
            double dlt_pref[DL_TOEP_PREF];
#pragma unroll
            for (int it = 0; it < DL_TOEP_PREF; ++it) dlt_pref[it] = (tid + it * nthr < o.n_t - 1) ? o.dlt[tid + it * nthr] : 0.;
            dl_fs_phase2_fir(tid, nthr, o, s);
            __syncthreads();
            if (stop_after == 2) return;
            dl_fs_phase2d_toep(tid, nthr, o, s, dlt_pref);
            __syncthreads();
            if (stop_after == 5) return;
        } else if (!o.fixed_spline) {
            dl_fs_phase2a(tid, nthr, o, s);
            __syncthreads();
            if (stop_after == 2) return;
            dl_fs_phase2b_dot(tid, nthr, o, s);
            __syncthreads();
            dl_fs_phase2b(tid, nthr, o, s);
            __syncthreads();
            if (stop_after == 3) return;
            dl_fs_phase2c_dot(tid, nthr, o, s);
            __syncthreads();
            dl_fs_phase2c(tid, nthr, o, s);
            __syncthreads();
            if (stop_after == 4) return;
            dl_fs_phase2d(tid, nthr, o, s);
            __syncthreads();
            if (stop_after == 5) return;
        }
    }
    double* prow = power + (size_t)b * (1 + o.n_var) * ld_power + o.col_offset;
    double* trow = tables ? tables + (size_t)b * ld_tables : nullptr;
    if (FAST && !EFT && !DENSE) dl_fs_phase3_pair<NL, EFT>(tid, nthr, o, s, lk_pref);
    else dl_fs_phase3<FAST, NL, EFT>(tid, nthr, o, s, trow, lk_pref);
    __syncthreads();
    DL_STAMP(4)
    dl_fs_phase4(tid, nthr, o, s, th, prow, ld_power);
    DL_STAMP(5)
    if (stamps != nullptr && threadIdx.x == 0) stamps[(size_t)blockIdx.x * 8 + 7] = __builtin_amdgcn_s_memrealtime();
#undef DL_STAMP
}

template <bool FAST, int NL, bool EFT, bool DENSE = false>
__global__ __launch_bounds__(DL_FS_THREADS, DENSE ? 5 : 4) void dl_fullshape_kernel(const DlObsDev o, const double* __restrict__ theta, int n_params, double* __restrict__ power,
                                                                     int64_t ld_power, double* __restrict__ tables, int64_t ld_tables, int stop_after, unsigned long long* __restrict__ stamps) {
    dl_obs_prefetch((const void*)__builtin_amdgcn_kernarg_segment_ptr());
    dl_fullshape_body<FAST, NL, EFT, DENSE>(o, theta, n_params, power, ld_power, tables, ld_tables, stop_after, stamps);
}

template <int NL>
__global__ __launch_bounds__(512, 2) void dl_fullshape_wide_kernel(const DlObsDev o, const double* __restrict__ theta, int n_params, double* __restrict__ power,
                                                                 int64_t ld_power, int stop_after, unsigned long long* __restrict__ stamps) {
    dl_obs_prefetch((const void*)__builtin_amdgcn_kernarg_segment_ptr());
    dl_fullshape_body<true, NL, false, false, false, false, 512>(o, theta, n_params, power, ld_power, nullptr, 0, stop_after, stamps);
}


__device__ __forceinline__ void dl_png_build_moments(int tid, int nthr, const DlObsDev& o, const DlFsShared& s, bool toep) {
    if (toep) {
        dl_fs_phase2_fir(tid, nthr, o, s);
    } else {
        dl_fs_phase2a(tid, nthr, o, s);
        __syncthreads();
        dl_fs_phase2b_dot(tid, nthr, o, s);
        __syncthreads();
        dl_fs_phase2b(tid, nthr, o, s);
        __syncthreads();
        dl_fs_phase2c_dot(tid, nthr, o, s);
        __syncthreads();
        dl_fs_phase2c(tid, nthr, o, s);
    }
    __syncthreads();
}

__global__ __launch_bounds__(DL_FS_THREADS, 2) void dl_png_kernel(DlObsDev o, const double* __restrict__ theta, int n_params, double* __restrict__ power, int64_t ld_power) {
    extern __shared__ __attribute__((aligned(16))) double lds[];
    const int tid = threadIdx.x, nthr = DL_FS_THREADS, n_t = o.n_t;
    const int64_t b = blockIdx.x;
    const double* th = theta + (size_t)b * n_params;
    const bool toep = o.toeplitz;
    const DlFsShared s = dl_fs_shared_carve(lds, n_t, o.n_in, -1, toep);
    double* tabs = s.coef;
    double* murec = lds + dl_fs_shared_doubles(n_t, o.n_in);
    double* sc = murec + 8 * DL_PNG_MAX_MU;
    dl_png_setup(tid, nthr, o, th, murec, sc);
    dl_png_knots(tid, nthr, o, th, s, true);
    __syncthreads();
    dl_png_build_moments(tid, nthr, o, s, toep);
    dl_png_keep_spline(tid, nthr, o, s, toep, tabs, tabs + n_t);
    __syncthreads();
    dl_png_knots(tid, nthr, o, th, s, false);
    __syncthreads();
    dl_png_build_moments(tid, nthr, o, s, toep);
    dl_png_keep_spline(tid, nthr, o, s, toep, tabs + 2 * n_t, tabs + 3 * n_t);
    __syncthreads();
    dl_png_eval(tid, nthr, o, tabs, murec, sc, s.out);
    __syncthreads();
    double* prow = power + (size_t)b * (1 + o.n_var) * ld_power + o.col_offset;
    for (int idx = tid; idx < o.n_in; idx += nthr) prow[idx] = s.out[idx];
}

template <bool FAST, int NL, bool EFT, bool DENSE = false>
__global__ __launch_bounds__(DL_FS_THREADS, DENSE ? 5 : 4) void dl_fullshape_multi_kernel(const DlObsDev* __restrict__ obs, const double* __restrict__ theta, int n_params,
                                                                           double* __restrict__ power, int64_t ld_power, int stop_after) {
    dl_fullshape_body<FAST, NL, EFT, DENSE>(obs[blockIdx.y], theta, n_params, power, ld_power, nullptr, 0, stop_after, nullptr);
}

#define DL_ENS_MAXP 32
#define DL_ENS_SLOTS_PER_WG 8
#define DL_EF_STAMP(slot) if (f.stamps != nullptr && publish && threadIdx.x == 0) { __builtin_amdgcn_s_waitcnt(0); f.stamps[(size_t)b * 8 + (slot)] = __builtin_amdgcn_s_memtime(); }
__device__ __forceinline__ void dl_ens_propose(const DlEnsFold& f, int b, bool publish, double* __restrict__ th_out, double* __restrict__ scratch) {
#pragma clang fp contract(off)
    const int lane = threadIdx.x & 63;
    DL_EF_STAMP(1)
    const int half = f.nw / 2, P = f.P;
    const DlPhilox r = dl_philox4x32((uint32_t)f.it_prop, (uint32_t)((unsigned long long)f.it_prop >> 32), (uint32_t)b, DL_ENS_STREAM_MOVE + f.half_prop, f.k0, f.k1);
    const double u = dl_uniform53(r.x[0], r.x[1]);
    const double t = (f.a - 1.) * u + 1.;
    const double zz = (t * t) / f.a;
    const int ic = dl_ens_split_at(f.split_prop, (1 - f.half_prop) * half + (int)(r.x[2] % (uint32_t)half));
    const int is = dl_ens_split_at(f.split_prop, f.half_prop * half + b);
    const int sA = dl_ens_pending_slot(f.pend, is, half), sB = dl_ens_pending_slot(f.pend, ic, half);
    const int p = lane < P ? lane : P - 1;
    DL_EF_STAMP(2)
    const double x_old = f.coords[(size_t)is * P + p], c_old = f.coords[(size_t)ic * P + p];
    const double x_new = f.pend.half >= 0 ? f.pend.prop[(size_t)(sA >= 0 ? sA : 0) * P + p] : 0., c_new = f.pend.half >= 0 ? f.pend.prop[(size_t)(sB >= 0 ? sB : 0) * P + p] : 0.;
    bool ax = false, ac = false;
    if (sA >= 0 || sB >= 0) {
        const DlEnsDecision2 d = dl_ens_decide2(f.pend, f.priors, P, f.n_tiles, f.offset, f.k0, f.k1, sA, f.logp[is], sB, f.logp[ic], scratch);
        ax = d.acc[0]; ac = d.acc[1];
    }
    DL_EF_STAMP(3)
    if (lane < P) {
        const double c = ac ? c_new : c_old, x = ax ? x_new : x_old;
        const double q = c - (c - x) * zz;
        th_out[lane] = q;
        if (publish) f.prop_out[(size_t)b * P + lane] = q;
    }
    if (publish && lane == 0) f.factors_out[b] = (P - 1.) * log(zz);
    DL_EF_STAMP(4)
}

__device__ __forceinline__ void dl_ens_write_state(const DlEnsFold& f, int e, double* __restrict__ scratch) {
#pragma clang fp contract(off)
    const int lane = threadIdx.x & 63, wave = threadIdx.x >> 6;
    const int half = f.nw / 2, P = f.P, hl = lane & 31, hb = lane >> 5;
    const int s0 = DL_ENS_SLOTS_PER_WG * e + 2 * wave, s1 = s0 + 1;
    if (s0 >= half) return;
    const bool two = s1 < half;
    const int w0 = dl_ens_split_at(f.pend.split, f.pend.half * half + s0), w1 = two ? dl_ens_split_at(f.pend.split, f.pend.half * half + s1) : w0;
    const double lw0 = f.logp[w0], lw1 = f.logp[w1];
    const int s = hb ? s1 : s0, w = hb ? w1 : w0;
    const int n = dl_ens_split_at(f.pend.split, (1 - f.pend.half) * half + (hb && !two ? s0 : s));
    const int p = hl < P ? hl : P - 1;
    const double v_old = f.coords[(size_t)w * P + p], v_new = f.pend.prop[(size_t)(hb && !two ? s0 : s) * P + p], v_n = f.coords[(size_t)n * P + p];
    const double ln = f.logp[n];
    const DlEnsDecision2 d = dl_ens_decide2(f.pend, f.priors, P, f.n_tiles, f.offset, f.k0, f.k1, s0, lw0, two ? s1 : -1, lw1, scratch + DL_ENS_SCRATCH * wave);
    if (hb && !two) return;
    const bool acc = hb ? d.acc[1] : d.acc[0];
    const double lp = hb ? d.lp[1] : d.lp[0], lw = hb ? lw1 : lw0;
    if (hl < P) {
        const double v = acc ? v_new : v_old;
        f.coords_out[(size_t)w * P + hl] = v; f.coords_out[(size_t)n * P + hl] = v_n;
        if (f.chain != nullptr) { f.chain[(size_t)w * P + hl] = v; f.chain[(size_t)n * P + hl] = v_n; }
    }
    if (hl == 0) {
        const double lv = acc ? lp : lw;
        f.logp_out[w] = lv; f.logp_out[n] = ln;
        if (acc) f.nacc[w] += 1;
        if (f.chain_logp != nullptr) { f.chain_logp[w] = lv; f.chain_logp[n] = ln; }
    }
}

template <int NL, bool DENSE = false>
__global__ __launch_bounds__(DL_FS_THREADS, DENSE ? 5 : 3) void dl_fullshape_ens_kernel(const DlObsDev* __restrict__ obs, const DlEnsFold f, double* __restrict__ power, int64_t ld_power,
                                                                         int flags, int B) {
    __shared__ double dl_ens_theta[DL_ENS_MAXP];
    __shared__ double dl_ens_scratch[DL_ENS_SCRATCH * (DL_FS_THREADS / 64)];
    const unsigned long long t_entry = __builtin_amdgcn_s_memtime();
    dl_kernarg_prefetch<(sizeof(DlEnsFold) + 8 + 63) / 64 * 64 + 64>();
    if ((int)blockIdx.x >= B) {
        if (blockIdx.y == 0 && f.pend.half >= 0) dl_ens_write_state(f, (int)blockIdx.x - B, dl_ens_scratch);
        return;
    }
    if (threadIdx.x < 64) dl_ens_propose(f, dl_fs_point_of_wg(blockIdx.x, (flags >> 8) & 0xff), blockIdx.y == 0, dl_ens_theta, dl_ens_scratch);
    else if (threadIdx.x < 128) {
        dl_scalar_prefetch<0, (offsetof(DlObsDev, ct_in) + 63) / 64 * 64, offsetof(DlObsDev, coef_w) / 64 * 64, (sizeof(DlObsDev) + 63) / 64 * 64>((const void*)(obs + blockIdx.y));
    }
    __syncthreads();
    if (f.stamps != nullptr && blockIdx.y == 0 && threadIdx.x == 0) { f.stamps[(size_t)dl_fs_point_of_wg(blockIdx.x, (flags >> 8) & 0xff) * 8 + 0] = t_entry; f.stamps[(size_t)dl_fs_point_of_wg(blockIdx.x, (flags >> 8) & 0xff) * 8 + 5] = __builtin_amdgcn_s_memtime(); }
    dl_fullshape_body<true, NL, false, DENSE, true>(obs[blockIdx.y], nullptr, f.P, power, ld_power, nullptr, 0, flags, nullptr, dl_ens_theta);
    if (f.stamps != nullptr && blockIdx.y == 0 && threadIdx.x == 0) f.stamps[(size_t)dl_fs_point_of_wg(blockIdx.x, (flags >> 8) & 0xff) * 8 + 6] = __builtin_amdgcn_s_memtime();
}

bool dl_launch_fullshape_ens(const DlObsDev* obs_host, int n_obs, const DlObsDev* obs_dev, const DlEnsFold& f, int64_t B, double* power, int64_t ld_power, int xcd_block, hipStream_t stream) {
    if (obs_dev == nullptr || n_obs < 1 || n_obs > 8 || f.P > DL_ENS_MAXP || f.P > 64) return false;
    const bool nl3 = obs_host[0].n_ell <= 3;
    size_t shmem = 0;
    for (int i = 0; i < n_obs; ++i) {
        const DlObsDev& oh = obs_host[i];
        const bool generic = !oh.uniform_knots || !(oh.toeplitz || oh.fixed_spline);
        if (oh.theory >= 2 || generic || oh.n_ct > 0 || oh.n_sn > 0 || (oh.n_ell <= 3) != nl3) return false;
        shmem = std::max(shmem, dl_fs_shared_doubles_obs(oh, true) * sizeof(double));
    }
    static const int64_t dense_min = getenv("DL_FS_DENSE_MIN") ? atoll(getenv("DL_FS_DENSE_MIN")) : 4096;
    auto launch = [&](auto kernel) {
        if (shmem > 48 * 1024) (void)hipFuncSetAttribute((const void*)kernel, hipFuncAttributeMaxDynamicSharedMemorySize, (int)shmem);
        const int flags = (xcd_block > 0 && B % (8 * xcd_block) == 0) ? (xcd_block << 8) : 0;
        const int n_extra = f.pend.half >= 0 ? (int)((B + DL_ENS_SLOTS_PER_WG - 1) / DL_ENS_SLOTS_PER_WG) : 0;
        DL_LAUNCH(kernel, dim3((unsigned)(B + n_extra), (unsigned)n_obs), dim3(DL_FS_THREADS), shmem, stream, obs_dev, f, power, ld_power, flags, (int)B);
    };
    if (nl3) { if (B * n_obs > dense_min) launch(dl_fullshape_ens_kernel<3, true>); else launch(dl_fullshape_ens_kernel<3>); }
    else { if (B * n_obs > dense_min) launch(dl_fullshape_ens_kernel<5, true>); else launch(dl_fullshape_ens_kernel<5>); }
    return true;
}

template <int NL>
__global__ __launch_bounds__(DL_FS_THREADS, 4) void dl_fullshape_grad_kernel(const DlObsDev* __restrict__ obs, const double* __restrict__ theta, int n_params,
                                                                              const double* __restrict__ Y, int64_t ldy, double* __restrict__ gphys) {
    extern __shared__ __attribute__((aligned(16))) double lds[];
    const DlObsDev& o = obs[blockIdx.y];
    const int b = blockIdx.x, tid = threadIdx.x, nthr = DL_FS_THREADS;
    constexpr int KT = DL_FS_KT;
    const double* th = theta + (size_t)b * n_params;
    const bool toep = o.toeplitz && !o.fixed_spline;
    const DlFsShared s = dl_fs_shared_carve(lds, o.n_t, o.n_in, dl_fs_n_dd0(o), toep);
    double* gw = s.pt + DL_PT_SIZE_FAST;
    double* red = gw + (size_t)DL_MAX_MU * DL_GW;
    auto build = [&]() {
        if (tid < KT) dl_fs_phase2_fir(tid, KT, o, s);
        __syncthreads();
        if (tid < KT) {
            double dlt_pref[DL_TOEP_PREF];
#pragma unroll
            for (int it = 0; it < DL_TOEP_PREF; ++it) dlt_pref[it] = (tid + it * KT < o.n_t - 1) ? o.dlt[tid + it * KT] : 0.;
            dl_fs_phase2d_toep(tid, KT, o, s, dlt_pref);
        }
        __syncthreads();
    };
    if (tid >= KT) {
        const int m = tid - KT;
        const bool mu_lane = m < o.n_mu;
        DlMuCarry c;
        dl_fs_mu_partA(o, th, mu_lane ? m : 0, c);
        dl_fs_mu_partB(c);
        if (mu_lane) { dl_fs_mu_partC(o, s, m, c, false); dl_fs_grad_weights(o, m, c, gw); }
        if (tid == nthr - 1) { dl_fs_scalars(o, th, s, c, false); dl_fs_grad_weights_pad(o, gw); }
    } else dl_fs_knots(tid, KT, o, th, s);
    __syncthreads();
    if (toep) build();
    double acc[DL_NPHYS];
#pragma unroll
    for (int p = 0; p < DL_NPHYS; ++p) acc[p] = 0.;
    const double* Yrow = Y + (size_t)b * ldy + o.col_offset;
    dl_fs_grad_phase3<NL>(tid, nthr, o, s, gw, Yrow, 0, acc);
    if (toep && o.templ == 1) {
        for (int which = 0; which < 2; ++which) {
            if (which == 0 ? o.dm.col < 0 : o.dn.col < 0) continue;
            __syncthreads();
            if (tid < KT) dl_fs_grad_knots(tid, KT, o, th, s, which);
            __syncthreads();
            build();
            dl_fs_grad_phase3<NL>(tid, nthr, o, s, gw, Yrow, 1 + which, acc);
        }
    }
#pragma unroll
    for (int p = 0; p < DL_NPHYS; ++p) {
        double v = acc[p];
#pragma unroll
        for (int off = 32; off >= 1; off >>= 1) v += __shfl_xor(v, off, 64);
        if ((tid & 63) == 0) red[(tid >> 6) * DL_NPHYS + p] = v;
    }
    __syncthreads();
    if (tid < DL_NPHYS) {
        double v = 0.;
#pragma unroll
        for (int w = 0; w < DL_FS_THREADS / 64; ++w) v += red[w * DL_NPHYS + tid];
        gphys[((size_t)b * gridDim.y + blockIdx.y) * DL_NPHYS + tid] = v;
    }
}

__global__ __launch_bounds__(64) void dl_grad_finalize_kernel(const DlObsDev* __restrict__ obs, int n_obs, const double* __restrict__ theta, int n_params, const double* __restrict__ priors,
                                                               const double* __restrict__ gphys, const int32_t* __restrict__ status, int64_t B, double* __restrict__ grad) {
    const int64_t b = (int64_t)blockIdx.x * blockDim.x + threadIdx.x;
    if (b >= B) return;
    const double* th = theta + (size_t)b * n_params;
    double* g = grad + (size_t)b * n_params;
    const bool ok = status == nullptr || status[b] == 0;
    for (int p = 0; p < n_params; ++p) {
        const double* pr = priors + 5 * p;
        g[p] = (ok && pr[0] == 1.) ? -(th[p] - pr[3]) / (pr[4] * pr[4]) : 0.;
    }
    if (!ok) return;
    for (int i = 0; i < n_obs; ++i) dl_fs_grad_chain(obs[i], th, gphys + ((size_t)b * n_obs + i) * DL_NPHYS, g);
}

// ... 30 lines not shown
    double* C = gw + (size_t)DL_MAX_MU * DL_GW;
    double* Jpoint = jac + (size_t)b * n_params * ldj;
    auto build = [&]() {
        if (tid < KT) dl_fs_phase2_fir(tid, KT, o, s);
        __syncthreads();
        if (tid < KT) {
            double dlt_pref[DL_TOEP_PREF];
#pragma unroll
            for (int it = 0; it < DL_TOEP_PREF; ++it) dlt_pref[it] = (tid + it * KT < o.n_t - 1) ? o.dlt[tid + it * KT] : 0.;
            dl_fs_phase2d_toep(tid, KT, o, s, dlt_pref);
        }
        __syncthreads();
    };
    if (tid >= KT) {
        const int m = tid - KT;
        const bool mu_lane = m < o.n_mu;
        DlMuCarry c;
        dl_fs_mu_partA(o, th, mu_lane ? m : 0, c);
        dl_fs_mu_partB(c);
        if (mu_lane) { dl_fs_mu_partC(o, s, m, c, false); dl_fs_grad_weights(o, m, c, gw); }
        if (tid == nthr - 1) { dl_fs_scalars(o, th, s, c, false); dl_fs_grad_weights_pad(o, gw); }
        dl_fs_jac_chain_matrix(m, o, th, n_params, C);
    } else dl_fs_knots(tid, KT, o, th, s);
    if (blockIdx.y == gridDim.y - 1) dl_fs_jac_zero_tail(tid, nthr, n_params, k_live, k_pad, Jpoint, ldj);
    __syncthreads();
    if (toep) build();
    double* J = Jpoint + o.col_offset;
    dl_fs_jac_phase3<NL, KPT>(tid, nthr, o, s, gw, C, n_params, 0, J, ldj);
    if (toep && o.templ == 1) {
        for (int which = 0; which < 2; ++which) {
            if (which == 0 ? o.dm.col < 0 : o.dn.col < 0) continue;
            __syncthreads();
            if (tid < KT) dl_fs_grad_knots(tid, KT, o, th, s, which);
            __syncthreads();
            build();
            dl_fs_jac_phase3<NL, KPT>(tid, nthr, o, s, gw, C, n_params, 1 + which, J, ldj);
        }
    }
}

void dl_launch_fullshape_jac(const DlObsDev* obs_host, int n_obs, const DlObsDev* obs_dev, const double* theta, int n_params, int64_t B, int k_live, int k_pad, double* jac, int64_t ldj,
                             hipStream_t stream) {
    size_t shm = 0;
    bool nl3 = true;
    for (int i = 0; i < n_obs; ++i) { shm = std::max(shm, dl_fs_jac_shared_doubles(obs_host[i], n_params) * sizeof(double)); nl3 = nl3 && obs_host[i].n_ell <= 3; }
    auto launch = [&](auto kernel) {
        if (shm > 48 * 1024) (void)hipFuncSetAttribute((const void*)kernel, hipFuncAttributeMaxDynamicSharedMemorySize, (int)shm);
        DL_LAUNCH(kernel, dim3((unsigned)B, (unsigned)n_obs), dim3(DL_FS_THREADS), shm, stream, obs_dev, theta, n_params, k_live, k_pad, jac, ldj);
    };
    if (nl3) launch(dl_fullshape_jac_kernel<3, 2>); else launch(dl_fullshape_jac_kernel<DL_MAX_ELL, 1>);
}

template <int MODEL>
__global__ __launch_bounds__(512) void dl_bao_kernel(const DlObsDev o, const double* __restrict__ theta, int n_params, double* __restrict__ power, int64_t ld_power) {
    extern __shared__ __attribute__((aligned(16))) double lds[];
    const int b = blockIdx.x, tid = threadIdx.x, nthr = blockDim.x;
    const double* th = theta + (size_t)b * n_params;
    dl_bao_phaseA(tid, nthr, o, th, lds);
    __syncthreads();
    dl_bao_phaseB_m<MODEL>(tid, nthr, o, lds);
    __syncthreads();
    dl_store_with_pass(tid, nthr, o, th, lds + DL_BAO_PT, power + (size_t)b * (1 + o.n_var) * ld_power + o.col_offset);
}

static int dl_bao_threads(int n_kin, int64_t B) {
    static const int forced = getenv("DL_BAO_THREADS") ? atoi(getenv("DL_BAO_THREADS")) : 0;
    if (forced >= 64 && forced <= 512 && forced % 64 == 0) return forced;
    int t = (n_kin + 63) / 64 * 64;
    t = t > 256 ? 256 : t;
    if (B >= 4096) t = 64;
    else if (B >= 2048 && t > 128) t = 128;
    return t;
}

__global__ __launch_bounds__(DL_FS_THREADS) void dl_emulated_kernel(const DlObsDev o, const double* __restrict__ theta, int n_params, double* __restrict__ power, int64_t ld_power,
                                                                   double* __restrict__ feat, int64_t feat_ld) {
    extern __shared__ __attribute__((aligned(16))) double lds[];
    const int b = blockIdx.x;
    dl_emu_point(o, theta + (size_t)b * n_params, lds, power + (size_t)b * (1 + o.n_var) * ld_power + o.col_offset, ld_power,
                 feat ? feat + (size_t)b * feat_ld + o.feat_off : nullptr);
}

void dl_launch_fullshape(const DlObsDev* obs_host, int n_obs, const double* theta, int n_params, int64_t B, double* power, int64_t ld_power, double* tables,
                         int64_t ld_tables, hipStream_t stream, double* feat, int64_t feat_ld, int xcd_block, const DlObsDev* obs_dev) {
    static const int stop_after = getenv("DL_FS_STOP") ? atoi(getenv("DL_FS_STOP")) : 0;
    static const char* stamp_file = getenv("DL_FS_STAMPS");
    static unsigned long long* stamps_dev = nullptr;
    static int stamp_launches = 0;
    if (stamp_file && !stamps_dev) { (void)hipMalloc((void**)&stamps_dev, (size_t)65536 * 8 * sizeof(unsigned long long)); }
    unsigned long long* stamps = (stamp_file && B >= 256 && B <= 65536 && stamp_launches >= 30 && stamp_launches < 34) ? stamps_dev : nullptr;
    if (stamp_file && B >= 256) stamp_launches++;
    const bool merge = !dl_options().no_merged_theory;
    if (merge && obs_dev != nullptr && n_obs > 1 && n_obs <= 8 && tables == nullptr && feat == nullptr && stop_after == 0 && !stamp_file) {
        bool same = true, eft0 = obs_host[0].n_ct > 0 || obs_host[0].n_sn > 0, nl3 = obs_host[0].n_ell <= 3;
        size_t shmem = 0;
        for (int i = 0; i < n_obs && same; ++i) {
            const DlObsDev& oh = obs_host[i];
            const bool generic = !oh.uniform_knots || !(oh.toeplitz || oh.fixed_spline);
            if (oh.theory >= 2 || generic || (oh.n_ct > 0 || oh.n_sn > 0) != eft0 || (oh.n_ell <= 3) != nl3) same = false;
            shmem = std::max(shmem, dl_fs_shared_doubles_obs(oh, true) * sizeof(double));
        }
        if (same && !eft0) {
            static const int64_t dense_min = getenv("DL_FS_DENSE_MIN") ? atoll(getenv("DL_FS_DENSE_MIN")) : 4096;
            auto launch = [&](auto kernel) {
                if (shmem > 48 * 1024) (void)hipFuncSetAttribute((const void*)kernel, hipFuncAttributeMaxDynamicSharedMemorySize, (int)shmem);
                const int flags = (xcd_block > 0 && B % (8 * xcd_block) == 0) ? (xcd_block << 8) : 0;
                DL_LAUNCH(kernel, dim3((unsigned)B, (unsigned)n_obs), dim3(DL_FS_THREADS), shmem, stream, obs_dev, theta, n_params, power, ld_power, flags);
            };
            if (nl3) { if (B * n_obs > dense_min) launch(dl_fullshape_multi_kernel<true, 3, false, true>); else launch(dl_fullshape_multi_kernel<true, 3, false>); }
            else { if (B * n_obs > dense_min) launch(dl_fullshape_multi_kernel<true, 5, false, true>); else launch(dl_fullshape_multi_kernel<true, 5, false>); }
            return;
        }
    }
    for (int i = 0; i < n_obs; ++i) {
        if (obs_host[i].theory == 5) {
            const size_t shm = dl_png_shared_doubles(obs_host[i].n_t, obs_host[i].n_in) * sizeof(double);
            if (shm > 48 * 1024) (void)hipFuncSetAttribute((const void*)dl_png_kernel, hipFuncAttributeMaxDynamicSharedMemorySize, (int)shm);
            DL_LAUNCH(dl_png_kernel, dim3((unsigned)B), dim3(DL_FS_THREADS), shm, stream, obs_host[i], theta, n_params, power, ld_power);
            continue;
        }
        if (obs_host[i].theory == 4) {
            dl_launch_tns(obs_host[i], theta, n_params, B, power, ld_power, stream);
            continue;
        }
        if (obs_host[i].theory == 3 && feat != nullptr && !dl_options().no_emu_batch) {
            size_t shm = dl_eb_shared_doubles(obs_host[i]) * sizeof(double);
            if (shm > 48 * 1024) (void)hipFuncSetAttribute((const void*)dl_emulated_batch_kernel, hipFuncAttributeMaxDynamicSharedMemorySize, (int)shm);
            DL_LAUNCH(dl_emulated_batch_kernel, dim3((unsigned)((B + DL_EB_PTS - 1) / DL_EB_PTS)), dim3(256), shm, stream, obs_host[i], theta, n_params, B, feat, feat_ld);
            continue;
        }
        if (obs_host[i].theory == 3) {
            size_t shm = dl_emu_shared_doubles_obs(obs_host[i]) * sizeof(double);
            DL_LAUNCH(dl_emulated_kernel, dim3((unsigned)B), dim3(DL_FS_THREADS), shm, stream, obs_host[i], theta, n_params, power, ld_power, feat, feat_ld);
            continue;
        }
        if (obs_host[i].theory == 2) {
            size_t shm = dl_bao_shared_doubles(obs_host[i].n_in) * sizeof(double);
            auto launch_bao = [&](auto kernel) {
                if (shm > 48 * 1024) (void)hipFuncSetAttribute((const void*)kernel, hipFuncAttributeMaxDynamicSharedMemorySize, (int)shm);
                DL_LAUNCH(kernel, dim3((unsigned)B), dim3((unsigned)dl_bao_threads(obs_host[i].n_kin, B)), shm, stream, obs_host[i], theta, n_params, power, ld_power);
            };
            const int model = obs_host[i].bao_mode >> 4;
            if (model == 0) launch_bao(dl_bao_kernel<0>);
            else if (model & 32) launch_bao(dl_bao_kernel<3>);
            else if (model & 16) launch_bao(dl_bao_kernel<2>);
            else launch_bao(dl_bao_kernel<1>);
            continue;
        }
        const DlObsDev& oh = obs_host[i];
        const bool generic = tables || !oh.uniform_knots || !(oh.toeplitz || oh.fixed_spline);
        size_t shmem = dl_fs_shared_doubles_obs(obs_host[i], !generic) * sizeof(double);
        auto launch = [&](auto kernel) {
            if (shmem > 48 * 1024) (void)hipFuncSetAttribute((const void*)kernel, hipFuncAttributeMaxDynamicSharedMemorySize, (int)shmem);
            const int flags = (xcd_block > 0 && stop_after == 0 && B % (8 * xcd_block) == 0) ? (xcd_block << 8) : stop_after;
            DL_LAUNCH(kernel, dim3((unsigned)B), dim3(DL_FS_THREADS), shmem, stream, obs_host[i], theta, n_params, power, ld_power, tables, ld_tables, flags, stamps);
            if (stamps) {
                (void)hipStreamSynchronize(stream);
                std::vector<unsigned long long> h((size_t)B * 8);
                (void)hipMemcpy(h.data(), stamps, h.size() * sizeof(unsigned long long), hipMemcpyDeviceToHost);
                if (FILE* f = fopen(stamp_file, "a")) {
                    for (int64_t w = 0; w < B; ++w) { for (int q = 0; q < 8; ++q) fprintf(f, "%llu ", h[(size_t)w * 8 + q]); fprintf(f, "\n"); }
                    fprintf(f, "#\n");
                    fclose(f);
                }
            }
        };
        static const int64_t dense_min = getenv("DL_FS_DENSE_MIN") ? atoll(getenv("DL_FS_DENSE_MIN")) : 4096;
        bool nl3 = oh.n_ell <= 3, eft = oh.n_ct > 0 || oh.n_sn > 0;
        static const int wide_env = getenv("DL_FS_WIDE") ? atoi(getenv("DL_FS_WIDE")) : -1;
        const bool wide = !generic && !eft && tables == nullptr && (wide_env == 1 || (wide_env != 0 && B * n_obs <= 256));
        if (wide) {
            if (shmem > 48 * 1024) { (void)hipFuncSetAttribute((const void*)dl_fullshape_wide_kernel<3>, hipFuncAttributeMaxDynamicSharedMemorySize, (int)shmem); (void)hipFuncSetAttribute((const void*)dl_fullshape_wide_kernel<5>, hipFuncAttributeMaxDynamicSharedMemorySize, (int)shmem); }
            const int flags = (xcd_block > 0 && stop_after == 0 && B % (8 * xcd_block) == 0) ? (xcd_block << 8) : stop_after;
            if (nl3) DL_LAUNCH(dl_fullshape_wide_kernel<3>, dim3((unsigned)B), dim3(512), shmem, stream, obs_host[i], theta, n_params, power, ld_power, flags, stamps);
            else DL_LAUNCH(dl_fullshape_wide_kernel<5>, dim3((unsigned)B), dim3(512), shmem, stream, obs_host[i], theta, n_params, power, ld_power, flags, stamps);
            continue;
        }
        if (generic) launch(dl_fullshape_kernel<false, 5, true>);
        else if (nl3 && !eft) { if (B > dense_min) launch(dl_fullshape_kernel<true, 3, false, true>); else launch(dl_fullshape_kernel<true, 3, false>); }
        else if (nl3) launch(dl_fullshape_kernel<true, 3, true>);
        else if (!eft) { if (B > dense_min) launch(dl_fullshape_kernel<true, 5, false, true>); else launch(dl_fullshape_kernel<true, 5, false>); }
        else launch(dl_fullshape_kernel<true, 5, true>);
    }
}

typedef double dl_double4 __attribute__((ext_vector_type(4)));
typedef double dl_double2 __attribute__((ext_vector_type(2)));

#define DL_GEMM_WAVES 8

struct DlGemmFrag {
    dl_double2 a[4], b0[4], b1[4];
};

__device__ __forceinline__ void dl_gemm_load(DlGemmFrag& f, const double* ap, const double* b0p, const double* b1p, int kc) {
    const dl_double2* a2 = reinterpret_cast<const dl_double2*>(ap + (size_t)kc * 32);
    const dl_double2* b02 = reinterpret_cast<const dl_double2*>(b0p + (size_t)kc * 32);
    const dl_double2* b12 = reinterpret_cast<const dl_double2*>(b1p + (size_t)kc * 32);
#pragma unroll
    for (int q = 0; q < 4; ++q) { f.a[q] = a2[4 * q]; f.b0[q] = b02[4 * q]; f.b1[q] = b12[4 * q]; }
}

__device__ __forceinline__ void dl_gemm_mma(const DlGemmFrag& f, dl_double4& acc0, dl_double4& acc1) {
#pragma unroll
    for (int q = 0; q < 4; ++q) {
        acc0 = __builtin_amdgcn_mfma_f64_16x16x4f64(f.a[q].x, f.b0[q].x, acc0, 0, 0, 0);
        acc1 = __builtin_amdgcn_mfma_f64_16x16x4f64(f.a[q].x, f.b1[q].x, acc1, 0, 0, 0);
        acc0 = __builtin_amdgcn_mfma_f64_16x16x4f64(f.a[q].y, f.b0[q].y, acc0, 0, 0, 0);
        acc1 = __builtin_amdgcn_mfma_f64_16x16x4f64(f.a[q].y, f.b1[q].y, acc1, 0, 0, 0);
    }
}

__global__ __launch_bounds__(64 * DL_GEMM_WAVES) void dl_window_gemm_kernel(const double* __restrict__ A, int64_t lda, const double* __restrict__ Wt, int64_t ldw,
                                                                            const double* __restrict__ bias, double* __restrict__ C, int64_t ldc, int M, int N_valid,
                                                                            int K_pad, int bias_period) {
    __shared__ __attribute__((aligned(16))) double red[DL_GEMM_WAVES - 1][2][4][64];
    const int lane = threadIdx.x & 63, wave = threadIdx.x >> 6;
    const int r16 = lane & 15, g = lane >> 4;
    const int m0 = blockIdx.x * 16, n0 = blockIdx.y * 32;
    int arow = m0 + r16;
    if (arow > M - 1) arow = M - 1;
    const double* ap = A + (size_t)arow * lda + g * 2;
    const double* b0p = Wt + (size_t)(n0 + r16) * ldw + g * 2;
    const double* b1p = Wt + (size_t)(n0 + 16 + r16) * ldw + g * 2;
    dl_double4 acc0 = {0., 0., 0., 0.}, acc1 = {0., 0., 0., 0.};
    const int nchunks = K_pad / 32;
    DlGemmFrag f0, f1;
    int kc = wave;
    if (kc < nchunks) dl_gemm_load(f0, ap, b0p, b1p, kc);
    for (; kc < nchunks; kc += 2 * DL_GEMM_WAVES) {
        int kn = kc + DL_GEMM_WAVES;
        if (kn < nchunks) dl_gemm_load(f1, ap, b0p, b1p, kn);
        dl_gemm_mma(f0, acc0, acc1);
        if (kn < nchunks) {
            int kn2 = kn + DL_GEMM_WAVES;
            if (kn2 < nchunks) dl_gemm_load(f0, ap, b0p, b1p, kn2);
            dl_gemm_mma(f1, acc0, acc1);
        }
    }
    if (wave > 0) {
#pragma unroll
        for (int r = 0; r < 4; ++r) { red[wave - 1][0][r][lane] = acc0[r]; red[wave - 1][1][r][lane] = acc1[r]; }
    }
    __syncthreads();
    if (wave == 0) {
#pragma unroll
        for (int r = 0; r < 4; ++r) {
            double s0 = acc0[r], s1 = acc1[r];
#pragma unroll
            for (int w = 0; w < DL_GEMM_WAVES - 1; ++w) { s0 += red[w][0][r][lane]; s1 += red[w][1][r][lane]; }
            int row = m0 + g + 4 * r;
            if (row < M) {
                bool wb = (row % bias_period) == 0;
                if (n0 + r16 < N_valid) C[(size_t)row * ldc + n0 + r16] = wb ? s0 + bias[n0 + r16] : s0;
                if (n0 + 16 + r16 < N_valid) C[(size_t)row * ldc + n0 + 16 + r16] = wb ? s1 + bias[n0 + 16 + r16] : s1;
            }
        }
    }
}

void dl_launch_window_gemm(const double* A, int64_t lda, const double* Wt, int64_t ldw, const double* bias, double* C, int64_t ldc, int64_t M, int N_valid, int N_pad,
                           int K_pad, int bias_period, hipStream_t stream) {
    dim3 grid((unsigned)((M + 15) / 16), (unsigned)(N_pad / 32));
    DL_LAUNCH(dl_window_gemm_kernel, grid, dim3(64 * DL_GEMM_WAVES), 0, stream, A, lda, Wt, ldw, bias, C, ldc, (int)M, N_valid, K_pad, bias_period);
// ... 1055 lines not shown
```

Measured before the change: 43.62 million evals/s.

## Add moment-form Hermite spline path with precomputed knot records in fullshape kernels

```diff
diff --git a/desilike_amd/csrc/dl_api.hip b/desilike_amd/csrc/dl_api.hip
--- a/desilike_amd/csrc/dl_api.hip
+++ b/desilike_amd/csrc/dl_api.hip
@@ -495,6 +495,7 @@
         if (k == "n_out_obs" + std::to_string(i)) return ctx->obs[i].n_out;
         if (k == "n_ell_obs" + std::to_string(i)) return ctx->obs[i].dev.n_ell;
         if (k == "n_kin_obs" + std::to_string(i)) return ctx->obs[i].dev.n_kin;
+        if (k == "moment_form_obs" + std::to_string(i)) return ctx->obs[i].dev.moment_form;
     }
     return -1;
 }
@@ -953,7 +954,8 @@
         const int64_t nb = std::min<int64_t>(per_pass, B - b0);
         const double* th = theta_dev + (size_t)b0 * P;
         int32_t* st = status_dev ? status_dev + b0 : ctx->grad_status;
-        dl_launch_fullshape(ctx->obs_kernarg.data(), ctx->n_obs, th, P, nb, ctx->power_ws, ctx->K_pad, nullptr, 0, stream, nullptr, 0, xcd_local ? dl_chi2_gemm_row_tile(nb, Np) : 0, ctx->obs_array_dev);
+        dl_launch_fullshape(ctx->obs_kernarg.data(), ctx->n_obs, th, P, nb, ctx->power_ws, ctx->K_pad, nullptr, 0, stream, nullptr, 0, xcd_local ? dl_chi2_gemm_row_tile(nb, Np) : 0, ctx->obs_array_dev,
+                            false);
         dl_launch_chi2_gemm(ctx->power_ws, Kp, ctx->wt_white_dev, Kp, ctx->bias_white_dev, ctx->delta_ws, nb, Np, Kp, nullptr, th, P, ctx->priors_dev, nullptr, nullptr, nullptr, 1, stream,
                             ctx->panel_ranges.empty() ? nullptr : ctx->panel_ranges.data(), ctx->K_live, ctx->grad_delta, Np, ctx->wt_frag_dev);
         dl_launch_finalize_part(ctx->delta_ws, Np / 16, th, P, ctx->priors_dev, nb, logposterior_dev + b0, nullptr, st, 1, stream);
diff --git a/desilike_amd/csrc/dl_fullshape.h b/desilike_amd/csrc/dl_fullshape.h
--- a/desilike_amd/csrc/dl_fullshape.h
+++ b/desilike_amd/csrc/dl_fullshape.h
@@ -65,7 +65,7 @@
     DlInput qpar, qper, qiso, qap, df, dm, dn, sigpar, sigper, b1X, b1Y, sn0;
     DlInput to_m, to_n, qto, dpto;
     double lkto_fid, lpkto_fid;
-    int32_t n_band, pad_band;
+    int32_t n_band, moment_form;
     DlInput band_in[DL_MAX_BAND];
     const double* band_tab;
     int32_t png_vel, pad_vel;
@@ -113,6 +113,7 @@
     const double *sp_A, *sp_nC, *sp_inv;
     const double *sp_gf, *sp_gb;
     const double *coef_fixed;
+    const double *knot_rec;
     const double *ct_matrix, *sn_matrix;
     DlInput sigmav, b2, bs, b3;
     void* tns_plan;
@@ -166,6 +167,23 @@
     return s;
 }
 
+DL_HD bool dl_fs_mom_direct(const DlObsDev& o) { return o.n_var == 0 && o.n_pass == 0; }
+DL_HD size_t dl_fs_mom_work_doubles(const DlObsDev& o) {
+    size_t w = (size_t)o.n_t + 2 * DL_FIR_PAD;
+    if (!dl_fs_mom_direct(o) && (size_t)o.n_in > w) w = (size_t)o.n_in;
+    return (w + 1) & ~(size_t)1;
+}
+DL_HD size_t dl_fs_mom_shared_doubles(const DlObsDev& o) { return 2 * (size_t)o.n_t + dl_fs_mom_work_doubles(o) + DL_PT_SIZE_FAST; }
+DL_HD DlFsShared dl_fs_shared_carve_mom(double* base, const DlObsDev& o) {
+    DlFsShared s;
+    s.coef = base;
+    double* work = base + 2 * (size_t)o.n_t;
+    s.y = work + DL_FIR_PAD; s.M = nullptr; s.z = nullptr;
+    s.out = work;
+    s.pt = work + dl_fs_mom_work_doubles(o);
+    return s;
+}
+
 DL_HD void dl_ap_qparqper(const DlObsDev& o, const double* th, double& qpar, double& qper) {
     switch (o.apmode) {
         case 1: qpar = qper = dl_get(o.qiso, th); break;
@@ -273,6 +291,19 @@
     } else {
         for (int j = tid; j < n_t; j += nthr) s.y[j] = o.pk_fid[j];
     }
+}
+
+#define DL_KNOT_PREF 3
+DL_HD void dl_fs_knots_rec(int tid, int nthr, const DlObsDev& o, const double* th, const DlFsShared& s, const double (*kr)[2]) {
+    const int n_t = o.n_t;
+    if (tid < 2 * DL_FIR_PAD) s.y[tid < DL_FIR_PAD ? tid - DL_FIR_PAD : n_t + tid - DL_FIR_PAD] = 0.;
+    const double dm_a = dl_get(o.dm, th) / o.a;
+#pragma unroll
+    for (int it = 0; it < DL_KNOT_PREF; ++it) {
+        const int j = tid + it * nthr;
+        if (j < n_t) s.y[j] = kr[it][0] * exp(dm_a * kr[it][1]);
+    }
+    for (int j = tid + DL_KNOT_PREF * nthr; j < n_t; j += nthr) s.y[j] = o.knot_rec[2 * j] * exp(dm_a * o.knot_rec[2 * j + 1]);
 }
 
 DL_HD void dl_fs_phase01(int tid, int nthr, const DlObsDev& o, const double* th, const DlFsShared& s) {
@@ -386,6 +417,7 @@
     }
 }
 
+template <bool MOM = false>
 DL_HD void dl_fs_phase2_fir(int tid, int nthr, const DlObsDev& o, const DlFsShared& s) {
     const double T[DL_FIR_D + 1] = DL_FIR_TAPS;
     const int n = o.n_t;
@@ -415,9 +447,15 @@
 #pragma unroll
             for (int c = 0; c < 4; ++c) cur[c] = nxt[c];
         }
-#pragma unroll
-        for (int q = 0; q < 4; ++q)
-            if (j0 + q < n) s.M[j0 + q] = acc[q] * scale;
+        if (MOM) {
+#pragma unroll
+            for (int q = 0; q < 4; ++q)
+                if (j0 + q < n) { s.coef[2 * (j0 + q)] = s.y[j0 + q]; s.coef[2 * (j0 + q) + 1] = acc[q]; }
+        } else {
+#pragma unroll
+            for (int q = 0; q < 4; ++q)
+                if (j0 + q < n) s.M[j0 + q] = acc[q] * scale;
+        }
     }
     for (int k = tid - (nthr - 2 * DL_FIR_PAD - 1); k >= 0 && k <= 2 * DL_FIR_PAD; k += nthr) {
         double v = exp((double)k * DL_FIR_LN_ABS_MU);
@@ -456,6 +494,39 @@
     }
 }
 
+#if defined(__HIPCC__)
+__device__ __forceinline__ void dl_fs_mom_fixup(int lane, const DlObsDev& o, const DlFsShared& s) {
+    const int n = o.n_t;
+    double* rec = s.coef;
+    const double a = ((rec[0] - rec[2]) - (rec[2] - rec[4])) * (1. / 6.) - rec[3];
+    const double b = ((rec[2 * (n - 3)] - rec[2 * (n - 2)]) - (rec[2 * (n - 2)] - rec[2 * (n - 1)])) * (1. / 6.) - rec[2 * (n - 2) + 1];
+    const bool left = lane < DL_FIR_PAD;
+    const int i = left ? 1 + lane : n - 2 - (lane - DL_FIR_PAD);
+    const int i2 = left ? i + 1 : i - 1;
+    const double mi = rec[2 * i + 1] + a * dl_fir_mu_pow(s, i - 1) + b * dl_fir_mu_pow(s, n - 2 - i);
+    const double mi2 = rec[2 * i2 + 1] + a * dl_fir_mu_pow(s, i2 - 1) + b * dl_fir_mu_pow(s, n - 2 - i2);
+    __asm__ volatile("s_waitcnt lgkmcnt(0)" : : : "memory");
+    rec[2 * i + 1] = mi;
+    if (lane == 0) rec[1] = o.end0a * mi + o.end0b * mi2;
+    if (lane == DL_FIR_PAD) rec[2 * (n - 1) + 1] = o.end1a * mi + o.end1b * mi2;
+}
+#endif
+
+DL_HD double dl_spline_eval_m(const DlObsDev& o, const DlFsShared& s, double t) {
+    int j = (int)t;
+#if defined(__HIP_DEVICE_COMPILE__)
+    __asm__("v_med3_i32 %0, %1, 0, %2" : "=v"(j) : "v"(j), "s"(o.n_t - 2));
+#else
+    j = j < 0 ? 0 : j;
+    if (j > o.n_t - 2) j = o.n_t - 2;
+#endif
+    const double u = t - (double)j;
+    const double* r = s.coef + 2 * j;
+    const double y0 = r[0], m0 = r[1], y1 = r[2], m1 = r[3];
+    const double c1 = (y1 - y0) - fma(2., m0, m1);
+    return fma(u, fma(u, fma(u, m1 - m0, 3. * m0), c1), y0);
+}
+
 template <bool UNIF>
 DL_HD void dl_spline_locate(const DlObsDev& o, double x, int& j, double& u) {
     const int n = o.n_t;
@@ -586,8 +657,8 @@
     }
 }
 
-template <int NL, bool EFT>
-DL_HD void dl_fs_phase3_pair(int tid, int nthr, const DlObsDev& o, const DlFsShared& s, const double* lk_pref = nullptr) {
+template <int NL, bool EFT, bool MOM = false>
+DL_HD void dl_fs_phase3_pair(int tid, int nthr, const DlObsDev& o, const DlFsShared& s, const double* lk_pref = nullptr, double* power_row = nullptr) {
     const double qper = s.pt[DL_PT_QPER], sn0nd = s.pt[DL_PT_SN0ND];
     const bool damp = s.pt[DL_PT_DAMP] != 0.;
     const bool need_dd0 = EFT && o.n_ct > 0;
@@ -608,7 +679,8 @@
                     for (int c = 0; c < o.n_sn; ++c) acc += o.sn_matrix[((size_t)l * n_kin + i) * o.n_sn + c] * s.pt[DL_PT_SN + c];
                     pl += acc;
                 }
-                s.out[(size_t)l * n_kin + i] = pl;
+                if (MOM && power_row != nullptr) DL_STREAM_STORE(&power_row[(size_t)l * n_kin + i], pl);
+                else s.out[(size_t)l * n_kin + i] = pl;
             }
         }
         if (EFT && o.n_var > 0) s.out[o.n_in + i] = dd0;
@@ -630,10 +702,10 @@
 #pragma unroll
             for (int q = 0; q < 4; ++q) lq[q] = s.pt[DL_PT_LQH + m0 + q];
 #pragma unroll
-            for (int q = 0; q < 4; ++q) TA[q] = dl_spline_eval_t(o, s, lkA + lq[q]);
+            for (int q = 0; q < 4; ++q) TA[q] = MOM ? dl_spline_eval_m(o, s, lkA + lq[q]) : dl_spline_eval_t(o, s, lkA + lq[q]);
             if (two) {
 #pragma unroll
-                for (int q = 0; q < 4; ++q) TB[q] = dl_spline_eval_t(o, s, lkB + lq[q]);
+                for (int q = 0; q < 4; ++q) TB[q] = MOM ? dl_spline_eval_m(o, s, lkB + lq[q]) : dl_spline_eval_t(o, s, lkB + lq[q]);
             } else {
 #pragma unroll
                 for (int q = 0; q < 4; ++q) TB[q] = 0.;
diff --git a/desilike_amd/csrc/dl_host.hpp b/desilike_amd/csrc/dl_host.hpp
--- a/desilike_amd/csrc/dl_host.hpp
+++ b/desilike_amd/csrc/dl_host.hpp
@@ -56,7 +56,7 @@
     std::vector<double> bias;
     std::vector<double> flatdata;
     size_t off_kin, off_lkin, off_mu, off_wmu, off_xt, off_pk, off_th, off_lg, off_ih, off_dlt, off_A, off_nC, off_inv, off_gf, off_gb, off_coef, off_ct, off_sn;
-    size_t off_cw, off_cn, off_pknowk, off_ml, off_pass, off_png = 0, off_band = 0;
+    size_t off_cw, off_cn, off_pknowk, off_ml, off_pass, off_png = 0, off_band = 0, off_krec = 0;
     size_t off_eng[3][6];
     size_t off_stk[3] = {0, 0, 0};
     int marg_vp[DL_N_VPARS];
@@ -67,7 +67,7 @@
         dev.kin = base + off_kin; dev.lkin = base + off_lkin; dev.mu = base + off_mu; dev.wmu = base + off_wmu;
         dev.x_t = base + off_xt; dev.pk_fid = base + off_pk; dev.sf_th = base + off_th; dev.sf_lg = base + off_lg;
         dev.ih = base + off_ih; dev.dlt = base + off_dlt; dev.sp_A = base + off_A; dev.sp_nC = base + off_nC; dev.sp_inv = base + off_inv;
-        dev.sp_gf = base + off_gf; dev.sp_gb = base + off_gb; dev.coef_fixed = base + off_coef;
+        dev.sp_gf = base + off_gf; dev.sp_gb = base + off_gb; dev.coef_fixed = base + off_coef; dev.knot_rec = base + off_krec;
         dev.ct_matrix = base + off_ct; dev.sn_matrix = base + off_sn;
         dev.coef_w = base + off_cw; dev.coef_n = base + off_cn; dev.pknow_k = base + off_pknowk; dev.ml_tab = base + off_ml; dev.pass_tab = base + off_pass; dev.png_alpha = base + off_png; dev.band_tab = base + off_band;
         for (int e = 0; e < 3; ++e) {
@@ -475,6 +475,24 @@
     d.toeplitz = (d.uniform_knots && d.n_t >= 4 * DL_FIR_PAD && !getenv("DL_NO_TOEPLITZ")) ? 1 : 0;
     for (int j = 0; j + 1 < d.n_t && d.toeplitz; ++j)
         if (std::fabs((x_t[j + 1] - x_t[j]) * d.inv_hx - 1.) > 1e-11) d.toeplitz = 0;
+    d.moment_form = 0;
+    std::vector<double> knot_rec(2, 0.);
+    if (d.toeplitz && !d.fixed_spline && d.templ == 1) {
+        double g = 4. * std::log(10.) / d.inv_hx, dmax = 0.;
+        double gfid = 0.;
+        for (int j = 0; j + 1 < d.n_t; ++j) {
+            const double r = (pk[j] > 0. && pk[j + 1] > 0.) ? std::fabs(std::log(pk[j + 1] / pk[j])) : HUGE_VAL;
+            if (!(r <= gfid)) gfid = r;
+        }
+        g += gfid;
+        for (int j = 0; j < d.n_t; ++j) dmax = std::max(dmax, std::fabs(dlt[j] * d.inv_hx));
+        if (g * dmax < 1e-14) d.moment_form = 1;
+        if (d.moment_form && d.dn.col < 0) {
+            knot_rec.resize((size_t)2 * d.n_t);
+            for (int j = 0; j < d.n_t; ++j) { knot_rec[2 * j] = pk[j] * std::exp(d.dn.value * sf_lg[j]); knot_rec[2 * j + 1] = sf_th[j]; }
+            d.moment_form |= 2;
+        }
+    }
     int m = d.n_t - 2;
     d.seg_warm = sp.warm;
     d.n_seg = DL_MAX_SEG;
@@ -589,7 +607,7 @@
     oh.off_kin = arena.push(kin); oh.off_lkin = arena.push(lkin); oh.off_mu = arena.push(mu); oh.off_wmu = arena.push(wmu);
     oh.off_xt = arena.push(x_t); oh.off_pk = arena.push(pk); oh.off_th = arena.push(sf_th); oh.off_lg = arena.push(sf_lg);
     oh.off_ih = arena.push(sp.ih); oh.off_dlt = arena.push(dlt); oh.off_A = arena.push(sp.A); oh.off_nC = arena.push(sp.nC); oh.off_inv = arena.push(sp.inv);
-    oh.off_gf = arena.push(gf); oh.off_gb = arena.push(gb); oh.off_coef = arena.push(coef);
+    oh.off_gf = arena.push(gf); oh.off_gb = arena.push(gb); oh.off_coef = arena.push(coef); oh.off_krec = arena.push(knot_rec);
     oh.off_ct = arena.push(ctm); oh.off_sn = arena.push(snm);
     oh.off_cw = arena.push(coef_w); oh.off_cn = arena.push(coef_n); oh.off_pknowk = arena.push(pknow_k);
     std::vector<double> png_alpha(2, 0.);
diff --git a/desilike_amd/csrc/dl_kernels.h b/desilike_amd/csrc/dl_kernels.h
--- a/desilike_amd/csrc/dl_kernels.h
+++ b/desilike_amd/csrc/dl_kernels.h
@@ -20,6 +20,7 @@
     int stk_overlap;
     bool ens_global, ens_force_comm, ens_no_defer, ens_no_fold, ens_stamps, ens_fold_stamps;
     bool no_emu_fused, no_gram_epilogue, step_kernel, chi2_fused, no_chi2_big;
+    bool fs_no_moments;
     int xcd_local;
     long long chi2_max_rows;
     int cg_mt;
@@ -34,7 +35,8 @@
 
 void dl_launch_fullshape(const DlObsDev* obs_host, int n_obs, const double* theta, int n_params, int64_t B, double* power, int64_t ld_power, double* tables,
                          int64_t ld_tables, hipStream_t stream, double* feat = nullptr, int64_t feat_ld = 0, int xcd_block = 0,
-                         const DlObsDev* obs_dev = nullptr);
+                         const DlObsDev* obs_dev = nullptr,
+                         bool moments = true);
 void dl_launch_window_gemm(const double* A, int64_t lda, const double* Wt, int64_t ldw, const double* bias, double* C, int64_t ldc, int64_t M, int N_valid, int N_pad,
                            int K_pad, int bias_period, hipStream_t stream);
 
diff --git a/desilike_amd/csrc/dl_kernels.hip b/desilike_amd/csrc/dl_kernels.hip
--- a/desilike_amd/csrc/dl_kernels.hip
+++ b/desilike_amd/csrc/dl_kernels.hip
@@ -43,6 +43,7 @@
     o.host_mode = std::getenv("DL_HOST_MODE") ? atoi(std::getenv("DL_HOST_MODE")) : -1;
     auto flag = [](const char* name) { const char* v = std::getenv(name); return v != nullptr && atoi(v) != 0; };
     o.no_emu_fused = on("DL_NO_EMU_FUSED"); o.no_gram_epilogue = on("DL_NO_GRAM_EPILOGUE"); o.no_chi2_big = on("DL_NO_CHI2_BIG");
+    o.fs_no_moments = flag("DL_FS_NO_MOMENTS");
     o.step_kernel = flag("DL_STEP_KERNEL"); o.chi2_fused = flag("DL_CHI2_FUSED"); o.chi2_bfrag = flag("DL_CHI2_BFRAG");
     o.xcd_local = std::getenv("DL_XCD_LOCAL") ? atoi(std::getenv("DL_XCD_LOCAL")) : 1;
     o.chi2_max_rows = std::getenv("DL_CHI2_GEMM_MAX") ? atoll(std::getenv("DL_CHI2_GEMM_MAX")) : 2048;
@@ -55,7 +56,7 @@
 
 __device__ __forceinline__ int dl_fs_point_of_wg(int wg, int xblk) { return xblk ? xblk * ((wg & 7) + 8 * ((wg >> 3) / xblk)) + ((wg >> 3) % xblk) : wg; }
 
-template <bool FAST, int NL, bool EFT, bool DENSE, bool TH_ROW = false, bool SUB = false, int NT = DL_FS_THREADS>
+template <bool FAST, int NL, bool EFT, bool DENSE, bool TH_ROW = false, bool SUB = false, int NT = DL_FS_THREADS, bool MOM = false>
 __device__ __forceinline__ void dl_fullshape_body(const DlObsDev& o, const double* __restrict__ theta, int n_params, double* __restrict__ power,
                                                   int64_t ld_power, double* __restrict__ tables, int64_t ld_tables, int stop_after, unsigned long long* __restrict__ stamps,
                                                   const double* th_row = nullptr,
@@ -69,7 +70,9 @@
     DL_STAMP(0)
     if (stamps != nullptr && threadIdx.x == 0) stamps[(size_t)blockIdx.x * 8 + 6] = __builtin_amdgcn_s_memrealtime();
     const bool toep = !o.fixed_spline && (FAST || o.toeplitz);
-    const DlFsShared s = dl_fs_shared_carve(lds, o.n_t, o.n_in, dl_fs_n_dd0(o), toep);
+    static_assert(!MOM || (FAST && !EFT && !DENSE), "the moment form belongs to the pair evaluation");
+    const DlFsShared s = MOM ? dl_fs_shared_carve_mom(lds, o) : dl_fs_shared_carve(lds, o.n_t, o.n_in, dl_fs_n_dd0(o), toep);
+    const bool direct = MOM && dl_fs_mom_direct(o);
     const double* th = TH_ROW ? th_row : theta + (size_t)b * n_params;
     const int tid = SUB ? tid_sub : (int)threadIdx.x, nthr = NT;
     if (stop_after == -1) return;
@@ -84,8 +87,17 @@
         DlMuCarry c;
         double dlt_pref[DL_TOEP_PREF];
 #pragma unroll
-        for (int it = 0; it < DL_TOEP_PREF; ++it) dlt_pref[it] = (toep && !mu_wave && tid + it * KT < o.n_t - 1) ? o.dlt[tid + it * KT] : 0.;
+        for (int it = 0; it < DL_TOEP_PREF; ++it) dlt_pref[it] = (!MOM && toep && !mu_wave && tid + it * KT < o.n_t - 1) ? o.dlt[tid + it * KT] : 0.;
+        const bool knot_rec = MOM && (o.moment_form & 2);
+        double kr[DL_KNOT_PREF][2];
+#pragma unroll
+        for (int it = 0; it < DL_KNOT_PREF; ++it) {
+            const bool live = knot_rec && !mu_wave && tid + it * KT < o.n_t;
+            const double2 r = live ? *reinterpret_cast<const double2*>(o.knot_rec + 2 * (size_t)(tid + it * KT)) : make_double2(0., 0.);
+            kr[it][0] = r.x; kr[it][1] = r.y;
+        }
         if (mu_wave) dl_fs_mu_partA(o, th, mu_lane ? m : 0, c);
+        else if (knot_rec) dl_fs_knots_rec(tid, KT, o, th, s, kr);
         else dl_fs_knots(tid, KT, o, th, s);
         if (o.fixed_spline && mu_wave) {
             dl_fs_mu_partB(c);
@@ -97,14 +109,15 @@
         if (stop_after == 1) return;
         if (toep) {
             if (mu_wave) dl_fs_mu_partB(c);
-            else dl_fs_phase2_fir(tid, KT, o, s);
+            else dl_fs_phase2_fir<MOM>(tid, KT, o, s);
             __syncthreads();
             DL_STAMP(2)
             if (stop_after == 2) return;
             if (mu_wave) {
                 if (mu_lane) dl_fs_mu_partC(o, s, m, c, false);
                 if (scalar_lane) dl_fs_scalars(o, th, s, c, false);
-            } else dl_fs_phase2d_toep(tid, KT, o, s, dlt_pref);
+            } else if (MOM) { if (tid < 64) dl_fs_mom_fixup(tid, o, s); }
+            else dl_fs_phase2d_toep(tid, KT, o, s, dlt_pref);
             __syncthreads();
             DL_STAMP(3)
             if (stop_after == 5) return;
@@ -144,28 +157,40 @@
     }
     double* prow = power + (size_t)b * (1 + o.n_var) * ld_power + o.col_offset;
     double* trow = tables ? tables + (size_t)b * ld_tables : nullptr;
-    if (FAST && !EFT && !DENSE) dl_fs_phase3_pair<NL, EFT>(tid, nthr, o, s, lk_pref);
+    if (FAST && !EFT && !DENSE) dl_fs_phase3_pair<NL, EFT, MOM>(tid, nthr, o, s, lk_pref, direct ? prow : nullptr);
     else dl_fs_phase3<FAST, NL, EFT>(tid, nthr, o, s, trow, lk_pref);
-    __syncthreads();
-    DL_STAMP(4)
-    dl_fs_phase4(tid, nthr, o, s, th, prow, ld_power);
+    if (!direct) {
+        __syncthreads();
+        DL_STAMP(4)
+        dl_fs_phase4(tid, nthr, o, s, th, prow, ld_power);
+    } else {
+        DL_STAMP(4)
+    }
     DL_STAMP(5)
     if (stamps != nullptr && threadIdx.x == 0) stamps[(size_t)blockIdx.x * 8 + 7] = __builtin_amdgcn_s_memrealtime();
 #undef DL_STAMP
 }
 
-template <bool FAST, int NL, bool EFT, bool DENSE = false>
+template <bool FAST, int NL, bool EFT, bool DENSE = false, bool MOM = false>
 __global__ __launch_bounds__(DL_FS_THREADS, DENSE ? 5 : 4) void dl_fullshape_kernel(const DlObsDev o, const double* __restrict__ theta, int n_params, double* __restrict__ power,
                                                                      int64_t ld_power, double* __restrict__ tables, int64_t ld_tables, int stop_after, unsigned long long* __restrict__ stamps) {
     dl_obs_prefetch((const void*)__builtin_amdgcn_kernarg_segment_ptr());
-    dl_fullshape_body<FAST, NL, EFT, DENSE>(o, theta, n_params, power, ld_power, tables, ld_tables, stop_after, stamps);
-}
-
-template <int NL>
+    dl_fullshape_body<FAST, NL, EFT, DENSE, false, false, DL_FS_THREADS, MOM>(o, theta, n_params, power, ld_power, tables, ld_tables, stop_after, stamps);
+}
+
+static bool dl_fs_use_moments(const DlObsDev* obs_host, int n_obs) {
+    if (dl_options().fs_no_moments) return false;
+    for (int i = 0; i < n_obs; ++i)
+        if (!(obs_host[i].moment_form & 1) || obs_host[i].n_ct > 0 || obs_host[i].n_sn > 0) return false;
+    return true;
+}
+static size_t dl_fs_fast_shared_bytes(const DlObsDev& oh, bool mom) { return (mom ? dl_fs_mom_shared_doubles(oh) : dl_fs_shared_doubles_obs(oh, true)) * sizeof(double); }
+
+template <int NL, bool MOM = false>
 __global__ __launch_bounds__(512, 2) void dl_fullshape_wide_kernel(const DlObsDev o, const double* __restrict__ theta, int n_params, double* __restrict__ power,
                                                                  int64_t ld_power, int stop_after, unsigned long long* __restrict__ stamps) {
     dl_obs_prefetch((const void*)__builtin_amdgcn_kernarg_segment_ptr());
-    dl_fullshape_body<true, NL, false, false, false, false, 512>(o, theta, n_params, power, ld_power, nullptr, 0, stop_after, stamps);
+    dl_fullshape_body<true, NL, false, false, false, false, 512, MOM>(o, theta, n_params, power, ld_power, nullptr, 0, stop_after, stamps);
 }
 
 
@@ -213,10 +238,10 @@
     for (int idx = tid; idx < o.n_in; idx += nthr) prow[idx] = s.out[idx];
 }
 
-template <bool FAST, int NL, bool EFT, bool DENSE = false>
+template <bool FAST, int NL, bool EFT, bool DENSE = false, bool MOM = false>
 __global__ __launch_bounds__(DL_FS_THREADS, DENSE ? 5 : 4) void dl_fullshape_multi_kernel(const DlObsDev* __restrict__ obs, const double* __restrict__ theta, int n_params,
                                                                            double* __restrict__ power, int64_t ld_power, int stop_after) {
-    dl_fullshape_body<FAST, NL, EFT, DENSE>(obs[blockIdx.y], theta, n_params, power, ld_power, nullptr, 0, stop_after, nullptr);
+    dl_fullshape_body<FAST, NL, EFT, DENSE, false, false, DL_FS_THREADS, MOM>(obs[blockIdx.y], theta, n_params, power, ld_power, nullptr, 0, stop_after, nullptr);
 }
 
 #define DL_ENS_MAXP 32
@@ -285,7 +310,7 @@
     }
 }
 
-template <int NL, bool DENSE = false>
+template <int NL, bool DENSE = false, bool MOM = false>
 __global__ __launch_bounds__(DL_FS_THREADS, DENSE ? 5 : 3) void dl_fullshape_ens_kernel(const DlObsDev* __restrict__ obs, const DlEnsFold f, double* __restrict__ power, int64_t ld_power,
                                                                          int flags, int B) {
     __shared__ double dl_ens_theta[DL_ENS_MAXP];
@@ -302,7 +327,7 @@
     }
     __syncthreads();
     if (f.stamps != nullptr && blockIdx.y == 0 && threadIdx.x == 0) { f.stamps[(size_t)dl_fs_point_of_wg(blockIdx.x, (flags >> 8) & 0xff) * 8 + 0] = t_entry; f.stamps[(size_t)dl_fs_point_of_wg(blockIdx.x, (flags >> 8) & 0xff) * 8 + 5] = __builtin_amdgcn_s_memtime(); }
-    dl_fullshape_body<true, NL, false, DENSE, true>(obs[blockIdx.y], nullptr, f.P, power, ld_power, nullptr, 0, flags, nullptr, dl_ens_theta);
+    dl_fullshape_body<true, NL, false, DENSE, true, false, DL_FS_THREADS, MOM>(obs[blockIdx.y], nullptr, f.P, power, ld_power, nullptr, 0, flags, nullptr, dl_ens_theta);
     if (f.stamps != nullptr && blockIdx.y == 0 && threadIdx.x == 0) f.stamps[(size_t)dl_fs_point_of_wg(blockIdx.x, (flags >> 8) & 0xff) * 8 + 6] = __builtin_amdgcn_s_memtime();
 }
 
@@ -314,17 +339,18 @@
         const DlObsDev& oh = obs_host[i];
         const bool generic = !oh.uniform_knots || !(oh.toeplitz || oh.fixed_spline);
         if (oh.theory >= 2 || generic || oh.n_ct > 0 || oh.n_sn > 0 || (oh.n_ell <= 3) != nl3) return false;
-        shmem = std::max(shmem, dl_fs_shared_doubles_obs(oh, true) * sizeof(double));
     }
     static const int64_t dense_min = getenv("DL_FS_DENSE_MIN") ? atoll(getenv("DL_FS_DENSE_MIN")) : 4096;
+    const bool dense = B * n_obs > dense_min, mom = !dense && dl_fs_use_moments(obs_host, n_obs);
+    for (int i = 0; i < n_obs; ++i) shmem = std::max(shmem, dl_fs_fast_shared_bytes(obs_host[i], mom));
     auto launch = [&](auto kernel) {
         if (shmem > 48 * 1024) (void)hipFuncSetAttribute((const void*)kernel, hipFuncAttributeMaxDynamicSharedMemorySize, (int)shmem);
         const int flags = (xcd_block > 0 && B % (8 * xcd_block) == 0) ? (xcd_block << 8) : 0;
         const int n_extra = f.pend.half >= 0 ? (int)((B + DL_ENS_SLOTS_PER_WG - 1) / DL_ENS_SLOTS_PER_WG) : 0;
         DL_LAUNCH(kernel, dim3((unsigned)(B + n_extra), (unsigned)n_obs), dim3(DL_FS_THREADS), shmem, stream, obs_dev, f, power, ld_power, flags, (int)B);
     };
-    if (nl3) { if (B * n_obs > dense_min) launch(dl_fullshape_ens_kernel<3, true>); else launch(dl_fullshape_ens_kernel<3>); }
-    else { if (B * n_obs > dense_min) launch(dl_fullshape_ens_kernel<5, true>); else launch(dl_fullshape_ens_kernel<5>); }
+    if (nl3) { if (dense) launch(dl_fullshape_ens_kernel<3, true>); else if (mom) launch(dl_fullshape_ens_kernel<3, false, true>); else launch(dl_fullshape_ens_kernel<3>); }
+    else { if (dense) launch(dl_fullshape_ens_kernel<5, true>); else if (mom) launch(dl_fullshape_ens_kernel<5, false, true>); else launch(dl_fullshape_ens_kernel<5>); }
     return true;
 }
 
@@ -521,7 +547,7 @@
 }
 
 void dl_launch_fullshape(const DlObsDev* obs_host, int n_obs, const double* theta, int n_params, int64_t B, double* power, int64_t ld_power, double* tables,
-                         int64_t ld_tables, hipStream_t stream, double* feat, int64_t feat_ld, int xcd_block, const DlObsDev* obs_dev) {
+                         int64_t ld_tables, hipStream_t stream, double* feat, int64_t feat_ld, int xcd_block, const DlObsDev* obs_dev, bool moments) {
     static const int stop_after = getenv("DL_FS_STOP") ? atoi(getenv("DL_FS_STOP")) : 0;
     static const char* stamp_file = getenv("DL_FS_STAMPS");
     static unsigned long long* stamps_dev = nullptr;
@@ -537,17 +563,18 @@
             const DlObsDev& oh = obs_host[i];
             const bool generic = !oh.uniform_knots || !(oh.toeplitz || oh.fixed_spline);
             if (oh.theory >= 2 || generic || (oh.n_ct > 0 || oh.n_sn > 0) != eft0 || (oh.n_ell <= 3) != nl3) same = false;
-            shmem = std::max(shmem, dl_fs_shared_doubles_obs(oh, true) * sizeof(double));
         }
         if (same && !eft0) {
             static const int64_t dense_min = getenv("DL_FS_DENSE_MIN") ? atoll(getenv("DL_FS_DENSE_MIN")) : 4096;
+            const bool dense = B * n_obs > dense_min, mom = moments && !dense && dl_fs_use_moments(obs_host, n_obs);
+            for (int i = 0; i < n_obs; ++i) shmem = std::max(shmem, dl_fs_fast_shared_bytes(obs_host[i], mom));
             auto launch = [&](auto kernel) {
                 if (shmem > 48 * 1024) (void)hipFuncSetAttribute((const void*)kernel, hipFuncAttributeMaxDynamicSharedMemorySize, (int)shmem);
                 const int flags = (xcd_block > 0 && B % (8 * xcd_block) == 0) ? (xcd_block << 8) : 0;
                 DL_LAUNCH(kernel, dim3((unsigned)B, (unsigned)n_obs), dim3(DL_FS_THREADS), shmem, stream, obs_dev, theta, n_params, power, ld_power, flags);
             };
-            if (nl3) { if (B * n_obs > dense_min) launch(dl_fullshape_multi_kernel<true, 3, false, true>); else launch(dl_fullshape_multi_kernel<true, 3, false>); }
-            else { if (B * n_obs > dense_min) launch(dl_fullshape_multi_kernel<true, 5, false, true>); else launch(dl_fullshape_multi_kernel<true, 5, false>); }
+            if (nl3) { if (dense) launch(dl_fullshape_multi_kernel<true, 3, false, true>); else if (mom) launch(dl_fullshape_multi_kernel<true, 3, false, false, true>); else launch(dl_fullshape_multi_kernel<true, 3, false>); }
+            else { if (dense) launch(dl_fullshape_multi_kernel<true, 5, false, true>); else if (mom) launch(dl_fullshape_multi_kernel<true, 5, false, false, true>); else launch(dl_fullshape_multi_kernel<true, 5, false>); }
             return;
         }
     }
@@ -588,7 +615,12 @@
         }
         const DlObsDev& oh = obs_host[i];
         const bool generic = tables || !oh.uniform_knots || !(oh.toeplitz || oh.fixed_spline);
-        size_t shmem = dl_fs_shared_doubles_obs(obs_host[i], !generic) * sizeof(double);
+        static const int64_t dense_min = getenv("DL_FS_DENSE_MIN") ? atoll(getenv("DL_FS_DENSE_MIN")) : 4096;
+        bool nl3 = oh.n_ell <= 3, eft = oh.n_ct > 0 || oh.n_sn > 0;
+        static const int wide_env = getenv("DL_FS_WIDE") ? atoi(getenv("DL_FS_WIDE")) : -1;
+        const bool wide = !generic && !eft && tables == nullptr && (wide_env == 1 || (wide_env != 0 && B * n_obs <= 256));
+        const bool mom = moments && !generic && !eft && (wide || B <= dense_min) && dl_fs_use_moments(&oh, 1);
+        size_t shmem = generic ? dl_fs_shared_doubles_obs(oh, false) * sizeof(double) : dl_fs_fast_shared_bytes(oh, mom);
         auto launch = [&](auto kernel) {
             if (shmem > 48 * 1024) (void)hipFuncSetAttribute((const void*)kernel, hipFuncAttributeMaxDynamicSharedMemorySize, (int)shmem);
             const int flags = (xcd_block > 0 && stop_after == 0 && B % (8 * xcd_block) == 0) ? (xcd_block << 8) : stop_after;
@@ -604,21 +636,20 @@
                 }
             }
         };
-        static const int64_t dense_min = getenv("DL_FS_DENSE_MIN") ? atoll(getenv("DL_FS_DENSE_MIN")) : 4096;
-        bool nl3 = oh.n_ell <= 3, eft = oh.n_ct > 0 || oh.n_sn > 0;
-        static const int wide_env = getenv("DL_FS_WIDE") ? atoi(getenv("DL_FS_WIDE")) : -1;
-        const bool wide = !generic && !eft && tables == nullptr && (wide_env == 1 || (wide_env != 0 && B * n_obs <= 256));
         if (wide) {
-            if (shmem > 48 * 1024) { (void)hipFuncSetAttribute((const void*)dl_fullshape_wide_kernel<3>, hipFuncAttributeMaxDynamicSharedMemorySize, (int)shmem); (void)hipFuncSetAttribute((const void*)dl_fullshape_wide_kernel<5>, hipFuncAttributeMaxDynamicSharedMemorySize, (int)shmem); }
-            const int flags = (xcd_block > 0 && stop_after == 0 && B % (8 * xcd_block) == 0) ? (xcd_block << 8) : stop_after;
-            if (nl3) DL_LAUNCH(dl_fullshape_wide_kernel<3>, dim3((unsigned)B), dim3(512), shmem, stream, obs_host[i], theta, n_params, power, ld_power, flags, stamps);
-            else DL_LAUNCH(dl_fullshape_wide_kernel<5>, dim3((unsigned)B), dim3(512), shmem, stream, obs_host[i], theta, n_params, power, ld_power, flags, stamps);
+            auto launch_wide = [&](auto kernel) {
+                if (shmem > 48 * 1024) (void)hipFuncSetAttribute((const void*)kernel, hipFuncAttributeMaxDynamicSharedMemorySize, (int)shmem);
+                const int flags = (xcd_block > 0 && stop_after == 0 && B % (8 * xcd_block) == 0) ? (xcd_block << 8) : stop_after;
+                DL_LAUNCH(kernel, dim3((unsigned)B), dim3(512), shmem, stream, obs_host[i], theta, n_params, power, ld_power, flags, stamps);
+            };
+            if (nl3) { if (mom) launch_wide(dl_fullshape_wide_kernel<3, true>); else launch_wide(dl_fullshape_wide_kernel<3>); }
+            else { if (mom) launch_wide(dl_fullshape_wide_kernel<5, true>); else launch_wide(dl_fullshape_wide_kernel<5>); }
             continue;
         }
         if (generic) launch(dl_fullshape_kernel<false, 5, true>);
-        else if (nl3 && !eft) { if (B > dense_min) launch(dl_fullshape_kernel<true, 3, false, true>); else launch(dl_fullshape_kernel<true, 3, false>); }
+        else if (nl3 && !eft) { if (B > dense_min) launch(dl_fullshape_kernel<true, 3, false, true>); else if (mom) launch(dl_fullshape_kernel<true, 3, false, false, true>); else launch(dl_fullshape_kernel<true, 3, false>); }
         else if (nl3) launch(dl_fullshape_kernel<true, 3, true>);
-        else if (!eft) { if (B > dense_min) launch(dl_fullshape_kernel<true, 5, false, true>); else launch(dl_fullshape_kernel<true, 5, false>); }
+        else if (!eft) { if (B > dense_min) launch(dl_fullshape_kernel<true, 5, false, true>); else if (mom) launch(dl_fullshape_kernel<true, 5, false, false, true>); else launch(dl_fullshape_kernel<true, 5, false>); }
         else launch(dl_fullshape_kernel<true, 5, true>);
     }
 }
```

Result: faster. 44.26 million evals/s (median of 6 runs) (+1.5%).
